# SCoulY/MuSCLe

Hardware: AMD Instinct MI355X
Metric: images/sec (whole node), MCL EfficientNet-B7 448x448 bs=32/GPU (higher is better)
Workload: dtype f32; 1 GPU; train_mcl.py loop body, step-A (epoch-4 gates: focal+softmargin+pairwise+ER+IMC, one backward, one Adam step), MuSCLe(efficientnet-b7, last_pooling=False, 21 classes), random-init weights; per_gpu_batch=32, global_batch=32, image=448x448, parallelism=single, optimizer=Adam(lr=1e-4, wd=5e-5) fused, launch=eager, weight-gradient GEMMs on a second stream

## Files before the change

### include/muscle_hip.h

```cpp
#ifndef MUSCLE_HIP_H
#define MUSCLE_HIP_H

#ifdef __cplusplus
extern "C" {
#endif

int mx_version(void);
int mx_abi_hash(void);
const char* mx_last_error(void);


int mx_pw_fwd_parts(int M, int N, int K);
int mx_pw_fwd(const float* A, int a_mode, const float* a_scale, const float* a_shift, const float* a_gate,
              int rows_per_sample, const float* W, float* C, int M, int K, int N, int lda, int ldc,
              const float* bias, const float* residual, int relu, float* stats, void* stream);

int mx_set_gemm_mode(int mode);
int mx_get_gemm_mode(void);
int mx_set_wgrad_kernel(int kernel, int groups);
int mx_get_wgrad_kernel(void);
int mx_gemm_uses_split(int kind, int M, int N, int K);

long mx_pw_planes_bytes(int N, int K);
int mx_pw_planes_tiles(int N, int K);
int mx_pw_planes_batch(const long* table, int n, int total_tiles, void* stream);
int mx_pw_fwd_uses_planes(int M, int K, int N);
int mx_pw_fwd_planes(const float* A, const void* Wplanes, float* C, int M, int K, int N, int lda, int ldc,
                     const float* bias, const float* residual, int relu, float* stats, void* stream);

int mx_transpose(const float* src, float* dst, int rows, int cols, void* stream);
int mx_transpose_batch(const long* table, int n, int total_tiles, void* stream);

int mx_pw_dgrad(const float* G, const float* W, float* dX, int M, int K, int N, int ldg, int ldx,
                const float* residual, void* stream);

int mx_pw_dgrad_bnbwd(const float* G, const float* X, const float* coef, const float* Wt, float* dX, float* dZ, int M, int K, int N,
                      int ldg, int ldx, const float* residual, void* stream);

int mx_pw_fwd_act_uses_planes(int M, int K, int N);
int mx_pw_fwd_planes_act(const float* A, const float* scale, const float* shift, const float* gate, int rows_per_sample,
                         const void* Wplanes, float* C, int M, int K, int N, int lda, int ldc, float* stats, void* stream);

int mx_pw_dgrad_bnbwd_planes(const float* G, const float* X, const float* coef, const void* WtPlanes, float* dX, int M, int K, int N,
                             int ldg, int ldx, const float* residual, void* stream);
int mx_pw_wgrad_tile_bnbwd_ok(int R, int Co, int Ci);
int mx_pw_wgrad_small_bnbwd_ok(int R, int Co, int Ci);
int mx_pw_wgrad_small_bnbwd(const float* G, const float* G2, const float* coef, const float* X, float* dW, int R, int Co, int Ci,
                            int ldg, int ldx, void* ws, long ws_bytes, void* stream);
int mx_pw_wgrad_tile_bnbwd(const float* G, const float* G2, const float* coef, const float* X, float* dW, int R, int Co, int Ci,
                           int ldg, int ldx, void* ws, long ws_bytes, void* stream);
int mx_pw_wgrad_tile_bnbwd_dz_ok(int R, int Co, int Ci, int ldg, int ldx);
int mx_pw_wgrad_tile_bnbwd_dz(const float* G, const float* G2, const float* coef, const float* X, float* dW, float* dz, int R, int Co,
                              int Ci, int ldg, int ldx, void* ws, long ws_bytes, void* stream);

long mx_pw_wgrad_ws(int R, int Co, int Ci);
int mx_pw_wgrad(const float* G, const float* X, int x_mode, const float* x_scale, const float* x_shift,
                const float* x_gate, int rows_per_sample, float* dW, int R, int Co, int Ci, int ldg, int ldx,
                void* ws, long ws_bytes, void* stream);

long mx_pw_wgrad_small_ws(int R, int Co, int Ci, int x_mode);
int mx_pw_wgrad_small(const float* G, const float* X, int x_mode, const float* x_scale, const float* x_shift,
                      const float* x_gate, int rows_per_sample, float* dW, int R, int Co, int Ci, int ldg, int ldx,
                      void* ws, long ws_bytes, void* stream);

long mx_pw_wgrad_tile_ws(int R, int Co, int Ci, int x_mode);
int mx_pw_wgrad_tile(const float* G, const float* X, int x_mode, const float* x_scale, const float* x_shift,
                     const float* x_gate, int rows_per_sample, float* dW, int R, int Co, int Ci, int ldg, int ldx,
                     void* ws, long ws_bytes, void* stream);

int mx_bgemm(int layout, const float* A, const float* B, float* C, int M, int N, int K, int lda, int ldb, int ldc,
             long sa, long sb, long sc, int batch, int relu, void* stream);


int mx_colreduce_parts(long rows, int C);
int mx_colstats(const float* X, long rows, int C, float* part, void* stream);

int mx_bn_finalize(const float* part, int P, int C, double count, const float* gamma, const float* beta, float* running_mean,
                   float* running_var, float momentum, float eps, int training, float* scale, float* shift,
                   float* mean, float* rstd, double* acc , void* stream);

int mx_fold_block(const float* We, const float* g0, const float* b0, const float* m0, const float* v0, float eps0,
                  const float* g1, const float* b1, const float* m1, const float* v1, float eps1,
                  const float* Wp, const float* g2, const float* b2, const float* m2, const float* v2, float eps2,
                  int Cin, int Cexp, int Cout, float* We_f, float* be, float* s1, float* t1, float* Wp_f, float* bp, void* stream);

int mx_bn_apply(const float* P, const float* scale, const float* shift, const float* row_scale, const float* residual,
                const float* gate, float* out, long rows, int C, int rows_per_sample, int act, void* stream);

int mx_bn_bwd_reduce(const float* G, const float* X, const float* row_scale, const float* gate, const float* gate_add,
                     const float* act_scale, const float* act_shift, long rows, int C, int rows_per_sample,
                     float* part, void* stream);

int mx_bn_bwd_finalize(const float* part, int P, int C, double count, const float* gamma, const float* mean, const float* rstd,
                       int training, float* dgamma, float* dbeta, float* c1, float* c2, float* c3, double* acc,
                       void* stream);

int mx_bn_bwd_apply(const float* G, const float* X, const float* row_scale, const float* gate, const float* gate_add,
                    const float* act_scale, const float* act_shift, const float* c1, const float* c2, const float* c3,
                    float* out, long rows, int C, int rows_per_sample, void* stream);

long mx_pool_ws(long rows, int C, int rows_per_sample, int planes);
int mx_pool_sum(const float* X, const float* G, const float* scale, const float* shift, int act, long rows, int C,
                int rows_per_sample, float* out, void* ws, long ws_bytes, void* stream);

int mx_se_bn1_pool(const float* dA, const float* X, const float* scale, const float* shift, long rows, int C, int rows_per_sample,
                   float* out5, void* ws, long ws_bytes, void* stream);
int mx_bn1_sums_finalize(const float* pooled5, const float* gate, const float* gh, const float* W1, float inv_hw, float* add,
                         int N, int C, int SQ, double count, const float* gamma, const float* mean, const float* rstd, int training,
                         float* dgamma, float* dbeta, float* c1, float* c2, float* c3, void* stream);


int mx_dwconv_fwd_parts(int N, int Ho, int Wo, int C, int S);
long mx_dwconv_fwd_ws(int N, int Ho, int Wo, int C, int S);
int mx_dwconv_fwd(const float* X, const float* scale, const float* shift, const float* W, float* Y, float* stats,
                  const float* pool_scale, const float* pool_shift, float* pooled, void* ws, long ws_bytes, int N,
                  int H, int Wd, int C, int K, int S, int pad_lo, int Ho, int Wo, void* stream);

int mx_dwconv_bwd_data(const float* dY, const float* W, const float* residual, float* dX, int N, int H, int Wd, int C,
                       int K, int S, int pad_lo, int Ho, int Wo, void* stream);

int mx_dwconv_bwd_weight_parts(int N, int Ho, int Wo, int C, int S);
int mx_dwconv_bwd_weight(const float* X, const float* scale, const float* shift, const float* dY, float* dW, float* dw_scratch,
                         int N, int H, int Wd, int C, int K, int S, int pad_lo, int Ho, int Wo, void* stream);

int mx_dwconv_bwd_fused_parts(int N, int H, int Wd, int C, int K);
int mx_dwconv_bwd_fused(const float* dA, const float* D, const float* gate, const float* add, const float* a1, const float* b1,
                        const float* c1, const float* c2, const float* c3, const float* X, const float* a0, const float* b0,
                        const float* W, const float* residual, float* gX, float* dW, float* dw_scratch, float* part, int N, int H,
                        int Wd, int C, int K, int pad_lo, void* stream);

int mx_dwconv_bwd_fused_bn0(const float* dA, const float* D, const float* gate, const float* add, const float* a1, const float* b1,
                            const float* c1, const float* c2, const float* c3, const float* X, const float* a0, const float* b0,
                            const float* W, float* gX, float* dW, float* dw_scratch, float* part, int N, int H, int Wd, int C, int K,
                            int pad_lo, void* ws, long ws_bytes, double count, const float* gamma, const float* mean, const float* rstd,
                            int training, float* dgamma, float* dbeta, float* o1, float* o2, float* o3, void* stream);

int mx_dwconv_bwd_fused_s2_parts(int N, int H, int Wd, int C, int K);
int mx_dwconv_bwd_fused_s2(const float* dA, const float* D, const float* gate, const float* add, const float* a1, const float* b1,
                           const float* c1, const float* c2, const float* c3, const float* X, const float* a0, const float* b0,
                           const float* W, float* gX, float* dW, float* dw_scratch, float* part, int N, int H, int Wd, int C, int K,
                           int pad_lo, int Ho, int Wo, void* stream);

int mx_dw_parts_reduce(const float* part, int P, int n, float* dW, void* stream);


int mx_se_fwd(const float* pooled_sum, float inv_hw, const float* W1, const float* b1, const float* W2, const float* b2,
              float* s, float* h, float* gate, int N, int C, int SQ, void* stream);

int mx_se_bwd(const float* ggate, const float* gate, const float* s, const float* h, const float* W2,
              float* dW1, float* db1, float* dW2, float* db2, float* gh, int N, int C,
              int SQ, void* stream);

int mx_se_bwd_gh(const float* ggate, const float* gate, const float* h, const float* W2, float* gh, int N, int C, int SQ,
                 void* stream);
int mx_se_bwd_params(const float* ggate, const float* gate, const float* s, const float* h, const float* gh, float* dW1, float* db1,
                     float* dW2, float* db2, int N, int C, int SQ, void* stream);

int mx_stem_im2col(const float* img, float* out, int N, int H, int W, int Ho, int Wo, int pad_lo, void* stream);


int mx_resize_nhwc(const float* src, float* dst, int N, int Hs, int Ws, int C, int Hd, int Wd, int ldd, int coff, int relu,
                   void* stream);

int mx_upsample_to_nchw(const float* src, float* dst, int N, int Hs, int Ws, int lds, int K, int Hd, int Wd, void* stream);

int mx_infer_accum(const float* src, float* acc, int h, int w, int lds, int K, int Hs, int Ws, int H, int W, int flip, void* stream);
int mx_infer_norm(float* acc, int channels, long HW, void* stream);

int mx_cam_infer(const long* passes, int npass, int lds, int K, int H, int W, const int* keep, int nkeep, float* out_cam,
                 float* out_sgc, void* stream);

int mx_seg_infer(const long* passes, int npass, int lds, int K, int H, int W, const float* cls_scale, unsigned char* pred,
                 float* prob, void* stream);
int mx_seg_confusion(const unsigned char* pred, const unsigned char* gt, int K, int H, int W, long long* counts, void* stream);

int mx_seg_infer_batch(const long* rows, int nrow, int B, int lds, int K, int H, int W, const float* cls_scale, unsigned char* pred,
                       float* prob, const unsigned char* gt, long long* counts, void* stream);

int mx_input_stage(const unsigned char* src, const int* jobs, float* dst, int n, int Hd, int Wd, void* stream);

int mx_color_jitter(unsigned char* src, const int* jobs, unsigned long long* sums, int n, int max_pixels, void* stream);
// ... 158 lines not shown
```

### muscle_amd/csrc/bn.hip

```cpp
#include "common.h"

struct ColGeom {
  int rows, C, c4;
  int tcols;
  int rpp;
  int rows_per_block;
  int rps;
};

static ColGeom col_geom(long rows, int C, int rps, long rows_limit ,
                        int groups = 1 , int planes = 1) {
  ColGeom g;
  g.rows = (int)rows; g.C = C; g.c4 = C / 4; g.rps = rps;
  {
    const int cand[] = {g.c4 <= 256 ? g.c4 : 256, 256, 192, 128, 96, 64, 48, 32};
    double best = -1.0;
    g.tcols = cand[0];
    for (int tc : cand) {
      if (tc > g.c4) continue;
      const double util = (double)g.c4 / (double)(cdiv(g.c4, tc) * tc) * (double)(256 / tc * tc) / 256.0;
      if (groups > 1 ? util > best - 1e-9 : util > best + 1e-9) { best = util; g.tcols = tc; }
    }
  }
  g.rpp = 256 / g.tcols;
// ... 145 lines not shown
}

template <class F, int NOUT, bool PER_SAMPLE, typename OutT>
static void launch_colreduce(const F& f, long rows, int C, int rps, OutT* o0, OutT* o1, hipStream_t st, void* ws = nullptr) {
  if (PER_SAMPLE) {
    dim3 grid;
    ColGeom g = pool_geom(rows, C, rps, &grid);
    hipLaunchKernelGGL((colreduce_kernel<F, NOUT, PER_SAMPLE, OutT>), grid, dim3(256), 0, st, f, g, o0, o1,
                       ws ? reinterpret_cast<float*>((char*)ws + MX_WS_COUNTER_BYTES) : nullptr, reinterpret_cast<unsigned*>(ws));
    return;
  }
  ColGeom g = col_geom(rows, C, rps, rows, 1);
  dim3 grid(cdiv(rows, g.rows_per_block), cdiv(g.c4, g.tcols), 1);
  hipLaunchKernelGGL((colreduce_kernel<F, NOUT, PER_SAMPLE, OutT>), grid, dim3(256), 0, st, f, g, o0, o1, (float*)nullptr, (unsigned*)nullptr);
}

struct GEff {
  const float* G; const float* X;
  const float* rs; const float* gate; const float* add;
  const float* a; const float* b;
  int C, rps;
  __device__ __forceinline__ void get(long r, int c, float4& g, float4& x) const {
    get_n(r, (int)((unsigned)r / (unsigned)rps), c, g, x);
  }
  __device__ __forceinline__ void get_n(long r, int n, int c, float4& g, float4& x) const {
    g = ld4(G + r * C + c);
    x = ld4(X + r * C + c);
    if (rs) { float s = rs[n]; g.x *= s; g.y *= s; g.z *= s; g.w *= s; }
    if (gate) {
      float4 gt = ld4(gate + (long)n * C + c), ad = ld4(add + (long)n * C + c);
      g.x = g.x * gt.x + ad.x; g.y = g.y * gt.y + ad.y; g.z = g.z * gt.z + ad.z; g.w = g.w * gt.w + ad.w;
    }
    if (a) {
      float4 aa = ld4(a + c), bb = ld4(b + c);
      g.x *= swish_gradf_(aa.x * x.x + bb.x); g.y *= swish_gradf_(aa.y * x.y + bb.y);
      g.z *= swish_gradf_(aa.z * x.z + bb.z); g.w *= swish_gradf_(aa.w * x.w + bb.w);
    }
  }
};

struct FBwdReduce {
  static constexpr bool kPipelined = false;
  GEff e;
  __device__ __forceinline__ void eval(long r, int c, float4& s0, float4& s1) const {
    float4 g, x;
    e.get(r, c, g, x);
    s0.x += g.x; s0.y += g.y; s0.z += g.z; s0.w += g.w;
    s1.x += g.x * x.x; s1.y += g.y * x.y; s1.z += g.z * x.z; s1.w += g.w * x.w;
  }
};

struct FStats {
  static constexpr bool kPipelined = false;
  const float* X; int C;
  __device__ __forceinline__ void eval(long r, int c, float4& s0, float4& s1) const {
    float4 x = ld4(X + r * C + c);
    s0.x += x.x; s0.y += x.y; s0.z += x.z; s0.w += x.w;
    s1.x += x.x * x.x; s1.y += x.y * x.y; s1.z += x.z * x.z; s1.w += x.w * x.w;
  }
};

struct FPool {
  static constexpr bool kPipelined = true;
  const float* X; const float* G; const float* a; const float* b; int C; int act;
  __device__ __forceinline__ float4 value(float4 x, int c) const {
    if (a) {
      float4 aa = ld4(a + c), bb = ld4(b + c);
      x.x = aa.x * x.x + bb.x; x.y = aa.y * x.y + bb.y; x.z = aa.z * x.z + bb.z; x.w = aa.w * x.w + bb.w;
    }
    if (act) { x.x = swishf_(x.x); x.y = swishf_(x.y); x.z = swishf_(x.z); x.w = swishf_(x.w); }
    return x;
  }
  __device__ __forceinline__ void eval(long r, int c, float4& s0, float4& s1) const {
    float4 x = value(ld4(X + r * C + c), c);
    if (G) {
      float4 g = ld4(G + r * C + c);
      x.x *= g.x; x.y *= g.y; x.z *= g.z; x.w *= g.w;
    }
    s0.x += x.x; s0.y += x.y; s0.z += x.z; s0.w += x.w;
  }
};

__global__ __launch_bounds__(256) void se_bn1_pool_kernel(const float* G, const float* X, const float* a, const float* b, ColGeom g,
                                                          float* out , long plane, float* scratch ,
                                                          unsigned* counters) {
  __shared__ float4 sm[5][256];
  __shared__ unsigned last_flag;
  const int tid = threadIdx.x;
  const int used = g.tcols * g.rpp;
  const int tc = tid % g.tcols, tr = tid / g.tcols;
  const int c4 = blockIdx.y * g.tcols + tc;
  const int sample = blockIdx.z;
  const long r0 = (long)sample * g.rps + (long)blockIdx.x * g.rows_per_block;
  const long r1 = min((long)(sample + 1) * g.rps, r0 + g.rows_per_block);
  float4 acc[5];
#pragma unroll
  for (int i = 0; i < 5; ++i) acc[i] = make_float4(0, 0, 0, 0);
  if (tid < used && c4 < g.c4) {
    const int c = 4 * c4;
    const float4 aa = ld4(a + c), bb = ld4(b + c);
#define SE1(f, x, ga)                                          \
      {                                                           \
        float z = aa.f * x.f + bb.f, sg = sigmoidf_(z);           \
        float act = z * sg, sp = sg * (1.f + z * (1.f - sg));     \
        acc[0].f += ga.f * act; acc[1].f += ga.f * sp; acc[2].f += sp; \
        acc[3].f += ga.f * sp * x.f; acc[4].f += sp * x.f;        \
      }
    long r = r0 + tr;
    for (; r + 3 * g.rpp < r1; r += 4 * g.rpp) {
      const float4 x0 = ld4(X + r * g.C + c), g0 = ld4(G + r * g.C + c);
      const float4 x1 = ld4(X + (r + g.rpp) * g.C + c), g1 = ld4(G + (r + g.rpp) * g.C + c);
      const float4 x2 = ld4(X + (r + 2 * g.rpp) * g.C + c), g2 = ld4(G + (r + 2 * g.rpp) * g.C + c);
      const float4 x3 = ld4(X + (r + 3 * g.rpp) * g.C + c), g3 = ld4(G + (r + 3 * g.rpp) * g.C + c);
      SE1(x, x0, g0) SE1(y, x0, g0) SE1(z, x0, g0) SE1(w, x0, g0)
      SE1(x, x1, g1) SE1(y, x1, g1) SE1(z, x1, g1) SE1(w, x1, g1)
      SE1(x, x2, g2) SE1(y, x2, g2) SE1(z, x2, g2) SE1(w, x2, g2)
      SE1(x, x3, g3) SE1(y, x3, g3) SE1(z, x3, g3) SE1(w, x3, g3)
    }
    for (; r + g.rpp < r1; r += 2 * g.rpp) {
      const float4 x0 = ld4(X + r * g.C + c), g0 = ld4(G + r * g.C + c);
      const float4 x1 = ld4(X + (r + g.rpp) * g.C + c), g1 = ld4(G + (r + g.rpp) * g.C + c);
      SE1(x, x0, g0) SE1(y, x0, g0) SE1(z, x0, g0) SE1(w, x0, g0)
      SE1(x, x1, g1) SE1(y, x1, g1) SE1(z, x1, g1) SE1(w, x1, g1)
    }
    for (; r < r1; r += g.rpp) {
      const float4 x0 = ld4(X + r * g.C + c), g0 = ld4(G + r * g.C + c);
      SE1(x, x0, g0) SE1(y, x0, g0) SE1(z, x0, g0) SE1(w, x0, g0)
    }
#undef SE1
  }
#pragma unroll
  for (int i = 0; i < 5; ++i) sm[i][tid] = acc[i];
  __syncthreads();
  const bool owner = tid < g.tcols && c4 < g.c4;
  const long off = (long)sample * g.C + 4 * c4;
  float* dst = gridDim.x == 1 ? out : scratch + (long)blockIdx.x * 5 * plane;
  if (owner) {
#pragma unroll
    for (int i = 0; i < 5; ++i) {
      float4 s0 = sm[i][tid];
      for (int k = 1; k < g.rpp; ++k) { float4 t0 = sm[i][tid + k * g.tcols]; s0.x += t0.x; s0.y += t0.y; s0.z += t0.z; s0.w += t0.w; }
      if (gridDim.x == 1) st4(dst + i * plane + off, s0);
      else mx_st4_wt(dst + i * plane + off, s0);
    }
  }
  if (gridDim.x == 1) return;
  if (!mx_last_arriver(counters + sample * gridDim.y + blockIdx.y, gridDim.x, &last_flag)) return;
  if (owner) {
#pragma unroll
    for (int i = 0; i < 5; ++i) st4(out + i * plane + off, ordered_sum4(scratch + i * plane + off, gridDim.x, 5 * plane));
  }
}

constexpr int BN_MAX_SLICES = 64;
__global__ __launch_bounds__(256) void bn_parts_reduce_kernel(const float* part, int P, int C, int rows_per_slice, double* acc) {
  __shared__ double sh[2][8][32];
  const int cl = threadIdx.x & 31, rl = threadIdx.x >> 5;
  const int c = blockIdx.x * 32 + cl;
  const int p0 = blockIdx.y * rows_per_slice, p1 = min(P, p0 + rows_per_slice);
  double a = 0.0, b = 0.0;
  if (c < C) {
    int p = p0 + rl;
    for (; p + 24 < p1; p += 32) {
      float a0 = part[(long)p * 2 * C + c], b0 = part[(long)p * 2 * C + C + c];
      float a1 = part[(long)(p + 8) * 2 * C + c], b1 = part[(long)(p + 8) * 2 * C + C + c];
      float a2 = part[(long)(p + 16) * 2 * C + c], b2 = part[(long)(p + 16) * 2 * C + C + c];
      float a3 = part[(long)(p + 24) * 2 * C + c], b3 = part[(long)(p + 24) * 2 * C + C + c];
      a += ((double)a0 + (double)a1) + ((double)a2 + (double)a3);
      b += ((double)b0 + (double)b1) + ((double)b2 + (double)b3);
    }
    for (; p < p1; p += 8) { a += (double)part[(long)p * 2 * C + c]; b += (double)part[(long)p * 2 * C + C + c]; }
  }
  sh[0][rl][cl] = a; sh[1][rl][cl] = b;
  __syncthreads();
  if (rl != 0 || c >= C) return;
  for (int i = 1; i < 8; ++i) { a += sh[0][i][cl]; b += sh[1][i][cl]; }
  acc[(long)blockIdx.y * 2 * C + c] = a;
  acc[(long)blockIdx.y * 2 * C + C + c] = b;
}

static int launch_parts_reduce(const float* part, int P, int C, double* acc, hipStream_t st) {
  int slices = P / 32;
  if (slices < 1) slices = 1;
  if (slices > BN_MAX_SLICES) slices = BN_MAX_SLICES;
  int rps = (P + slices - 1) / slices;
  slices = (P + rps - 1) / rps;
  hipLaunchKernelGGL(bn_parts_reduce_kernel, dim3(cdiv(C, 32), slices), dim3(256), 0, st, part, P, C, rps, acc);
  return slices;
}

struct BnFwdFin {
  double count; const float* gamma; const float* beta; float* rmean; float* rvar; float momentum, eps; int training;
  float* scale; float* shift; float* mean_out; float* rstd_out;
};

__device__ __forceinline__ void bn_fwd_finalize_one(int c, double st0, double st1, double count, const float* gamma,
                                                    const float* beta, float* rmean, float* rvar, float momentum, float eps,
                                                    int training, float* scale, float* shift, float* mean_out, float* rstd_out) {
  float mean, rstd;
  if (training) {
    double m = st0 / count;
    double var = st1 / count - m * m;
    if (var < 0) var = 0;
    mean = (float)m;
    rstd = (float)(1.0 / sqrt(var + (double)eps));
    double unb = count > 1 ? var * count / (count - 1) : var;
    rmean[c] = (1.f - momentum) * rmean[c] + momentum * mean;
    rvar[c] = (1.f - momentum) * rvar[c] + momentum * (float)unb;
  } else {
    mean = rmean[c];
    rstd = 1.0f / sqrtf(rvar[c] + eps);
  }
  float sc = gamma[c] * rstd;
  scale[c] = sc;
  shift[c] = beta[c] - mean * sc;
  mean_out[c] = mean;
  rstd_out[c] = rstd;
}

__device__ __forceinline__ bool slices_sum(const double* acc, int slices, int C, double& s0, double& s1) {
  __shared__ double sh[2][8][32];
  const int cl = threadIdx.x & 31, sl = threadIdx.x >> 5;
  const int c = blockIdx.x * 32 + cl;
  s0 = s1 = 0.0;
  if (c < C)
    for (int i = sl; i < slices; i += 8) { s0 += acc[(long)i * 2 * C + c]; s1 += acc[(long)i * 2 * C + C + c]; }
  sh[0][sl][cl] = s0; sh[1][sl][cl] = s1;
  __syncthreads();
  if (sl != 0 || c >= C) return false;
  for (int i = 1; i < 8; ++i) { s0 += sh[0][i][cl]; s1 += sh[1][i][cl]; }
  return true;
}

__global__ __launch_bounds__(256) void bn_finalize_kernel(const double* acc, int slices, int C, double count, const float* gamma,
                                   const float* beta, float* rmean, float* rvar, float momentum, float eps, int training,
                                   float* scale, float* shift, float* mean_out, float* rstd_out) {
  double st0, st1;
  if (!slices_sum(acc, training ? slices : 0, C, st0, st1)) return;
  const int c = blockIdx.x * 32 + (threadIdx.x & 31);
  bn_fwd_finalize_one(c, st0, st1, count, gamma, beta, rmean, rvar, momentum, eps, training, scale, shift, mean_out, rstd_out);
}


__global__ __launch_bounds__(256) void bn_bwd_finalize_kernel(const double* acc, int slices, int C, double count, const float* gamma,
                                       const float* mean, const float* rstd, int training, float* dgamma, float* dbeta,
                                       float* c1, float* c2, float* c3) {
  double s0, s1;
  if (!slices_sum(acc, slices, C, s0, s1)) return;
  const int c = blockIdx.x * 32 + (threadIdx.x & 31);
  bn_bwd_finalize_one(c, s0, s1, count, gamma, mean, rstd, training, dgamma, dbeta, c1, c2, c3);
}

constexpr int FUSED_FINALIZE_MAX_ROWS = 1024;
template <bool BWD>
__global__ __launch_bounds__(256) void bn_reduce_finalize_kernel(const float* part, int P, int C, BnFwdFin f, BnBwdFin b) {
  __shared__ double sh[2][8][32];
  const int cl = threadIdx.x & 31, rl = threadIdx.x >> 5;
  const int c = blockIdx.x * 32 + cl;
  double s0 = 0.0, s1 = 0.0;
  if (c < C) bn_parts_lane_sum(part, P, C, c, rl, s0, s1);
  sh[0][rl][cl] = s0; sh[1][rl][cl] = s1;
  __syncthreads();
  if (rl != 0 || c >= C) return;
  for (int i = 1; i < 8; ++i) { s0 += sh[0][i][cl]; s1 += sh[1][i][cl]; }
  if (BWD) bn_bwd_finalize_one(c, s0, s1, b.count, b.gamma, b.mean, b.rstd, b.training, b.dgamma, b.dbeta, b.c1, b.c2, b.c3);
  else bn_fwd_finalize_one(c, s0, s1, f.count, f.gamma, f.beta, f.rmean, f.rvar, f.momentum, f.eps, 1, f.scale, f.shift, f.mean_out, f.rstd_out);
}

constexpr int B1_NL = 16;
template <bool STAGED>
__global__ __launch_bounds__(64 * B1_NL) void bn1_sums_finalize_kernel(const float* pooled , const float* gate, const float* gh,
                                                                      const float* W1, float inv_hw, float* add, int N, int C, int SQ,
                                                                      BnBwdFin b) {
  extern __shared__ float smem_b1[];
  const int cl = threadIdx.x & 63, nl = threadIdx.x >> 6;
  const int c = blockIdx.x * 64 + cl;
  const float* ghs = STAGED ? smem_b1 : gh;
  if (STAGED) {
    for (int i = threadIdx.x; i < N * SQ; i += 64 * B1_NL) smem_b1[i] = gh[i];
    __syncthreads();
  }
  const long plane = (long)N * C;
  double s0 = 0.0, s1 = 0.0;
  if (c < C) {
    for (int n0 = nl; n0 < N; n0 += 2 * B1_NL) {
      const int n1 = n0 + B1_NL;
      float a0 = 0.f, a1 = 0.f;
      const float* g0 = ghs + n0 * SQ;
      const float* g1 = ghs + (n1 < N ? n1 : n0) * SQ;
      int j = 0;
      for (; j + 32 <= SQ; j += 32) {
        float w[32];
#pragma unroll
        for (int u = 0; u < 32; ++u) w[u] = W1[(long)(j + u) * C + c];
        __builtin_amdgcn_sched_barrier(0);
#pragma unroll
        for (int u = 0; u < 32; ++u) { a0 += g0[j + u] * w[u]; a1 += g1[j + u] * w[u]; }
      }
      for (; j + 8 <= SQ; j += 8) {
        float w[8];
#pragma unroll
        for (int u = 0; u < 8; ++u) w[u] = W1[(long)(j + u) * C + c];
        __builtin_amdgcn_sched_barrier(0);
#pragma unroll
        for (int u = 0; u < 8; ++u) { a0 += g0[j + u] * w[u]; a1 += g1[j + u] * w[u]; }
      }
// ... 86 lines not shown
  float eps0, eps1, eps2;
  int Cin, Cexp, Cout;
  float *We_f, *be, *s1, *t1, *Wp_f, *bp;
};
__global__ __launch_bounds__(256) void fold_block_kernel(FoldArgs a) {
  const long tid = (long)blockIdx.x * 256 + threadIdx.x, nth = (long)gridDim.x * 256;
  if (a.We) {
    for (long i = tid; i < (long)a.Cexp * a.Cin; i += nth) {
      const int c = (int)(i / a.Cin);
      a.We_f[i] = a.We[i] * (a.g0[c] * rsqrtf(a.v0[c] + a.eps0));
    }
    for (long c = tid; c < a.Cexp; c += nth) {
      const float s = a.g0[c] * rsqrtf(a.v0[c] + a.eps0);
      a.be[c] = a.b0[c] - s * a.m0[c];
    }
  }
  for (long c = tid; c < a.Cexp; c += nth) {
    const float s = a.g1[c] * rsqrtf(a.v1[c] + a.eps1);
    a.s1[c] = s; a.t1[c] = a.b1[c] - s * a.m1[c];
  }
  for (long i = tid; i < (long)a.Cout * a.Cexp; i += nth) {
    const int c = (int)(i / a.Cexp);
    a.Wp_f[i] = a.Wp[i] * (a.g2[c] * rsqrtf(a.v2[c] + a.eps2));
  }
  for (long c = tid; c < a.Cout; c += nth) {
    const float s = a.g2[c] * rsqrtf(a.v2[c] + a.eps2);
    a.bp[c] = a.b2[c] - s * a.m2[c];
  }
}

extern "C" {

int mx_fold_block(const float* We, const float* g0, const float* b0, const float* m0, const float* v0, float eps0,
                  const float* g1, const float* b1, const float* m1, const float* v1, float eps1,
                  const float* Wp, const float* g2, const float* b2, const float* m2, const float* v2, float eps2,
                  int Cin, int Cexp, int Cout, float* We_f, float* be, float* s1, float* t1, float* Wp_f, float* bp, void* stream) {
  MX_CHECK_ARG(Cin > 0 && Cexp > 0 && Cout > 0, "fold_block: bad extents");
  MX_CHECK_ARG(!We || (g0 && b0 && m0 && v0 && We_f && be), "fold_block: expand weight without its BatchNorm / outputs");
  MX_CHECK_ARG(g1 && b1 && m1 && v1 && s1 && t1 && Wp && g2 && b2 && m2 && v2 && Wp_f && bp, "fold_block: null pointer");
  FoldArgs a{We, g0, b0, m0, v0, g1, b1, m1, v1, Wp, g2, b2, m2, v2, eps0, eps1, eps2, Cin, Cexp, Cout, We_f, be, s1, t1, Wp_f, bp};
  long work = (long)Cexp * (Cin > Cout ? Cin : Cout);
  int grid = (int)((work + 1023) / 1024);
  if (grid > 1024) grid = 1024;
  if (grid < 1) grid = 1;
  hipLaunchKernelGGL(fold_block_kernel, dim3(grid), dim3(256), 0, (hipStream_t)stream, a);
  MX_LAUNCH_CHECK();
  return MX_OK;
}

int mx_colreduce_parts(long rows, int C) {
  if (rows <= 0 || C <= 0 || C % 4) return MX_EARG;
  return colreduce_parts(rows, C);
}

int mx_colstats(const float* X, long rows, int C, float* part, void* stream) {
  MX_CHECK_ARG(X && part && rows > 0 && C > 0 && C % 4 == 0, "colstats: bad args rows=%ld C=%d", rows, C);
  FStats f{X, C};
  launch_colreduce<FStats, 2, false, float>(f, rows, C, 1, part, part, (hipStream_t)stream);
  MX_LAUNCH_CHECK();
  return MX_OK;
}

int mx_bn_finalize(const float* part, int P, int C, double count, const float* gamma, const float* beta, float* running_mean,
                   float* running_var, float momentum, float eps, int training, float* scale, float* shift,
                   float* mean, float* rstd, double* acc, void* stream) {
  MX_CHECK_ARG(C > 0 && gamma && beta && running_mean && running_var && scale && shift && mean && rstd,
               "bn_finalize: null argument");
  MX_CHECK_ARG(!training || (part && P > 0 && count > 0 && acc), "bn_finalize: training needs partial statistics, count and acc[64][2C]");
  if (training && P <= FUSED_FINALIZE_MAX_ROWS) {
    BnFwdFin f{count, gamma, beta, running_mean, running_var, momentum, eps, 1, scale, shift, mean, rstd};
    hipLaunchKernelGGL(bn_reduce_finalize_kernel<false>, dim3(cdiv(C, 32)), dim3(256), 0, (hipStream_t)stream, part, P, C, f, BnBwdFin{});
    MX_LAUNCH_CHECK();
    return MX_OK;
  }
  int slices = 0;
  if (training) slices = launch_parts_reduce(part, P, C, acc, (hipStream_t)stream);
  hipLaunchKernelGGL(bn_finalize_kernel, dim3(cdiv(C, 32)), dim3(256), 0, (hipStream_t)stream, acc, slices, C, count, gamma,
                     beta, running_mean, running_var, momentum, eps, training, scale, shift, mean, rstd);
  MX_LAUNCH_CHECK();
  return MX_OK;
}

int mx_bn_apply(const float* P, const float* scale, const float* shift, const float* row_scale, const float* residual,
                const float* gate, float* out, long rows, int C, int rows_per_sample, int act, void* stream) {
  MX_CHECK_ARG(P && scale && shift && out && rows > 0 && C % 4 == 0 && rows_per_sample > 0, "bn_apply: bad args");
  long total4 = rows * (C / 4);
  hipLaunchKernelGGL(bn_apply_kernel, dim3(grid_for(total4)), dim3(256), 0, (hipStream_t)stream, P, scale, shift,
                     row_scale, residual, gate, out, total4, C, rows_per_sample, act);
  MX_LAUNCH_CHECK();
  return MX_OK;
}

int mx_bn_bwd_reduce(const float* G, const float* X, const float* row_scale, const float* gate, const float* gate_add,
                     const float* act_scale, const float* act_shift, long rows, int C, int rows_per_sample,
                     float* part, void* stream) {
  MX_CHECK_ARG(G && X && part && rows > 0 && C % 4 == 0 && rows_per_sample > 0, "bn_bwd_reduce: bad args");
  MX_CHECK_ARG((gate == nullptr) == (gate_add == nullptr), "bn_bwd_reduce: gate and gate_add come together");
  MX_CHECK_ARG((act_scale == nullptr) == (act_shift == nullptr), "bn_bwd_reduce: act scale/shift come together");
  FBwdReduce f{GEff{G, X, row_scale, gate, gate_add, act_scale, act_shift, C, rows_per_sample}};
  launch_colreduce<FBwdReduce, 2, false, float>(f, rows, C, rows_per_sample, part, part, (hipStream_t)stream);
  MX_LAUNCH_CHECK();
  return MX_OK;
}

int mx_bn_bwd_finalize(const float* part, int P, int C, double count, const float* gamma, const float* mean, const float* rstd,
                       int training, float* dgamma, float* dbeta, float* c1, float* c2, float* c3, double* acc, void* stream) {
  MX_CHECK_ARG(part && P > 0 && gamma && mean && rstd && dgamma && dbeta && c1 && c2 && c3 && acc && C > 0 && count > 0,
               "bn_bwd_finalize: bad args");
  if (P <= FUSED_FINALIZE_MAX_ROWS) {
    BnBwdFin b{count, gamma, mean, rstd, training, dgamma, dbeta, c1, c2, c3};
    hipLaunchKernelGGL(bn_reduce_finalize_kernel<true>, dim3(cdiv(C, 32)), dim3(256), 0, (hipStream_t)stream, part, P, C, BnFwdFin{}, b);
    MX_LAUNCH_CHECK();
    return MX_OK;
  }
  const int slices = launch_parts_reduce(part, P, C, acc, (hipStream_t)stream);
  hipLaunchKernelGGL(bn_bwd_finalize_kernel, dim3(cdiv(C, 32)), dim3(256), 0, (hipStream_t)stream, acc, slices, C, count, gamma,
                     mean, rstd, training, dgamma, dbeta, c1, c2, c3);
  MX_LAUNCH_CHECK();
  return MX_OK;
}

int mx_bn_bwd_apply(const float* G, const float* X, const float* row_scale, const float* gate, const float* gate_add,
                    const float* act_scale, const float* act_shift, const float* c1, const float* c2, const float* c3,
                    float* out, long rows, int C, int rows_per_sample, void* stream) {
  MX_CHECK_ARG(G && X && out && c1 && c2 && c3 && rows > 0 && C % 4 == 0 && rows_per_sample > 0, "bn_bwd_apply: bad args");
  GEff e{G, X, row_scale, gate, gate_add, act_scale, act_shift, C, rows_per_sample};
  long total4 = rows * (C / 4);
  hipLaunchKernelGGL(bn_bwd_apply_kernel, dim3(grid_for(total4)), dim3(256), 0, (hipStream_t)stream, e, c1, c2, c3, out,
                     total4);
  MX_LAUNCH_CHECK();
  return MX_OK;
}

long mx_pool_ws(long rows, int C, int rows_per_sample, int planes) {
  if (rows <= 0 || C <= 0 || C % 4 || rows_per_sample <= 0 || rows % rows_per_sample || (planes != 1 && planes != 5)) return MX_EARG;
  return pool_ws_bytes(rows, C, rows_per_sample, planes);
}

int mx_se_bn1_pool(const float* dA, const float* X, const float* scale, const float* shift, long rows, int C, int rows_per_sample,
                   float* out5, void* ws, long ws_bytes, void* stream) {
  MX_CHECK_ARG(dA && X && scale && shift && out5 && rows > 0 && C % 4 == 0 && rows_per_sample > 0 && rows % rows_per_sample == 0,
               "se_bn1_pool: bad args");
  const int N = (int)(rows / rows_per_sample);
  dim3 grid;
  ColGeom g = pool_geom(rows, C, rows_per_sample, &grid, 5);
  const long need = pool_ws_bytes(rows, C, rows_per_sample, 5);
  MX_CHECK_ARG(need == 0 || (ws && ws_bytes >= need && ((uintptr_t)ws & 15) == 0), "se_bn1_pool: workspace of %ld bytes required (mx_pool_ws)", need);
  hipLaunchKernelGGL(se_bn1_pool_kernel, grid, dim3(256), 0, (hipStream_t)stream, dA, X, scale, shift, g, out5, (long)N * C,
                     need ? reinterpret_cast<float*>((char*)ws + MX_WS_COUNTER_BYTES) : nullptr, reinterpret_cast<unsigned*>(ws));
  MX_LAUNCH_CHECK();
  return MX_OK;
}

int mx_bn1_sums_finalize(const float* pooled5, const float* gate, const float* gh, const float* W1, float inv_hw, float* add,
                         int N, int C, int SQ, double count, const float* gamma, const float* mean, const float* rstd, int training,
                         float* dgamma, float* dbeta, float* c1, float* c2, float* c3, void* stream) {
  MX_CHECK_ARG(pooled5 && gate && gh && W1 && add && N > 0 && C > 0 && SQ > 0 && count > 0, "bn1_sums_finalize: bad args");
  MX_CHECK_ARG(gamma && mean && rstd && dgamma && dbeta && c1 && c2 && c3, "bn1_sums_finalize: null pointer");
  const size_t redb = 2 * B1_NL * 64 * sizeof(double);
  const size_t shb = (size_t)((N * SQ + 1) & ~1) * sizeof(float) + redb;
  BnBwdFin b{count, gamma, mean, rstd, training, dgamma, dbeta, c1, c2, c3};
  if (shb <= 64 * 1024)
    hipLaunchKernelGGL(bn1_sums_finalize_kernel<true>, dim3(cdiv(C, 64)), dim3(64 * B1_NL), shb, (hipStream_t)stream, pooled5, gate, gh, W1,
                       inv_hw, add, N, C, SQ, b);
  else
    hipLaunchKernelGGL(bn1_sums_finalize_kernel<false>, dim3(cdiv(C, 64)), dim3(64 * B1_NL), redb, (hipStream_t)stream, pooled5, gate, gh, W1,
                       inv_hw, add, N, C, SQ, b);
  MX_LAUNCH_CHECK();
  return MX_OK;
}

int mx_pool_sum(const float* X, const float* G, const float* scale, const float* shift, int act, long rows, int C,
                int rows_per_sample, float* out, void* ws, long ws_bytes, void* stream) {
  MX_CHECK_ARG(X && out && rows > 0 && C % 4 == 0 && rows_per_sample > 0 && rows % rows_per_sample == 0,
               "pool_sum: bad args rows=%ld C=%d rps=%d", rows, C, rows_per_sample);
  const long need = pool_ws_bytes(rows, C, rows_per_sample, 1);
  MX_CHECK_ARG(need == 0 || (ws && ws_bytes >= need && ((uintptr_t)ws & 15) == 0), "pool_sum: workspace of %ld bytes required (mx_pool_ws)", need);
  FPool f{X, G, scale, shift, C, act};
  launch_colreduce<FPool, 1, true, float>(f, rows, C, rows_per_sample, out, out, (hipStream_t)stream, need ? ws : nullptr);
  MX_LAUNCH_CHECK();
  return MX_OK;
}

}
```

### muscle_amd/csrc/gemm.hip

```cpp
#include "common.h"
#include <type_traits>
#include <stdlib.h>

typedef float f32x16 __attribute__((ext_vector_type(16)));
typedef float f32x4 __attribute__((ext_vector_type(4)));

struct GemmArgs {
  MxOperand a, b;
  float* c;
  int M, N, K;
  int lda, ldb, ldc;
  long sa, sb, sc;
  const float* bias;
  const float* residual;
  int relu;
  float* stats;
  int ksplit;
  int xcd_nt;
  int mt, zt;
  unsigned long long* stamps;
  float* a_out;
  float* ws;
};

#ifndef MX_GEMM_STAMP
#define MX_GEMM_STAMP(g, slot)
#endif
static unsigned long long* mx_gemm_stamps = nullptr;

enum { L_NT = 0, L_NN = 1, L_TN = 2 };

template <int ROWS, int PAD, int BK>
struct SlabK {
  static constexpr int TOTAL = ROWS * (BK / 4);
  static constexpr int PER = (TOTAL + 255) / 256;
  float4 v[PER];
  __device__ __forceinline__ void load(const MxOperand& o, const float* base, int ld, int r0, int rows_total,
                                       int k0, int K, int tid) {
#pragma unroll
    for (int i = 0; i < PER; ++i) {
      int idx = tid + 256 * i;
      int k4 = idx % (BK / 4), row = idx / (BK / 4);
      int r = r0 + row, k = k0 + 4 * k4;
      float4 x = make_float4(0.f, 0.f, 0.f, 0.f);
      if (idx < TOTAL && r < rows_total && k < K) {
        x = ld4(base + (long)r * ld + k);
        x = mx_apply(o, x, r, k, K);
      }
      v[i] = x;
    }
  }
  __device__ __forceinline__ void store(float* lds, int tid) const {
#pragma unroll
    for (int i = 0; i < PER; ++i) {
      int idx = tid + 256 * i;
      int k4 = idx % (BK / 4), row = idx / (BK / 4);
      if (idx < TOTAL) {
        float* p = lds + (4 * k4) * (ROWS + PAD) + row;
        p[0] = v[i].x; p[ROWS + PAD] = v[i].y; p[2 * (ROWS + PAD)] = v[i].z; p[3 * (ROWS + PAD)] = v[i].w;
      }
    }
  }
};

template <int COLS, int PAD, int BK>
struct SlabN {
  static constexpr int C4 = COLS / 4;
  static constexpr int TOTAL = BK * C4;
  static constexpr int PER = (TOTAL + 255) / 256;
  float4 v[PER];
  __device__ __forceinline__ void load(const MxOperand& o, const float* base, int ld, int c0, int cols_total,
                                       int k0, int Kdim, int tid) {
#pragma unroll
    for (int i = 0; i < PER; ++i) {
      int idx = tid + 256 * i;
      int c4 = idx % C4, kk = idx / C4;
      int k = k0 + kk, c = c0 + 4 * c4;
      float4 x = make_float4(0.f, 0.f, 0.f, 0.f);
      if (idx < TOTAL && k < Kdim && c < cols_total) {
        x = ld4(base + (long)k * ld + c);
        x = mx_apply(o, x, k, c, cols_total);
      }
      v[i] = x;
    }
  }
  __device__ __forceinline__ void store(float* lds, int tid) const {
#pragma unroll
    for (int i = 0; i < PER; ++i) {
      int idx = tid + 256 * i;
      int c4 = idx % C4, kk = idx / C4;
      if (idx < TOTAL) st4(lds + kk * (COLS + PAD) + 4 * c4, v[i]);
    }
  }
};

constexpr int gemm_min_waves(int acc_regs, int bk) { return (acc_regs == 64 && bk == 16) ? 4 : 1; }

template <int LAYOUT, int WM, int WN, int TM, int TN, int BK>
__global__ __launch_bounds__(256, gemm_min_waves(TM * TN * 16, BK)) void gemm_kernel(GemmArgs g) {
  constexpr int BM = WM * TM * 32, BN = WN * TN * 32;
  constexpr int PADA = (LAYOUT == L_TN) ? 4 : 1;
  constexpr int PADB = (LAYOUT == L_NT) ? 1 : 4;
  constexpr int SA = BM + PADA, SB = BN + PADB;
  __shared__ __attribute__((aligned(16))) float smem[2 * BK * SA + 2 * BK * SB];
  float* As = smem;
  float* Bs = smem + 2 * BK * SA;

  const int tid = threadIdx.x, lane = tid & 63, wave = tid >> 6;
  const int l31 = lane & 31, h = lane >> 5;
  const int wm = wave / WN, wn = wave % WN;
  int tile_m = blockIdx.x, tile_n = blockIdx.y;
  int zz = blockIdx.z;
  if (LAYOUT == L_TN && g.xcd_nt > 0) {
    const int L = blockIdx.x, xcd = L & 7, j = L >> 3;
    const int tiles = g.mt * g.xcd_nt;
    const int t = j % tiles;
    zz = (j / tiles) * 8 + xcd;
    if (zz >= g.zt) return;
    tile_m = t % g.mt; tile_n = t / g.mt;
  } else if (g.xcd_nt > 0) {
    const int L = blockIdx.x, xcd = L & 7, j = L >> 3;
    tile_n = j % g.xcd_nt;
    tile_m = (j / g.xcd_nt) * 8 + xcd;
    if (tile_m >= g.mt) return;
  }
  const int m0 = tile_m * BM, n0 = tile_n * BN;
  const int z = zz;

  const float* A = g.a.p;
  const float* B = g.b.p;
  float* C = g.c;
  int kbeg = 0, kend = g.K;
  if (LAYOUT == L_TN) {
    kbeg = z * g.ksplit;
    kend = min(g.K, kbeg + g.ksplit);
    C += z * g.sc;
  } else {
    A += z * g.sa; B += z * g.sb; C += z * g.sc;
  }

  f32x16 acc[TM][TN];
#pragma unroll
  for (int i = 0; i < TM; ++i)
#pragma unroll
    for (int j = 0; j < TN; ++j)
#pragma unroll
      for (int r = 0; r < 16; ++r) acc[i][j][r] = 0.f;

  typename std::conditional<LAYOUT == L_TN, SlabN<BM, PADA, BK>, SlabK<BM, PADA, BK>>::type sa;
  typename std::conditional<LAYOUT == L_NT, SlabK<BN, PADB, BK>, SlabN<BN, PADB, BK>>::type sb;

  auto load = [&](int k0) {
    if constexpr (LAYOUT == L_TN) sa.load(g.a, A, g.lda, m0, g.M, k0, kend, tid);
    else sa.load(g.a, A, g.lda, m0, g.M, k0, kend, tid);
    if constexpr (LAYOUT == L_NT) sb.load(g.b, B, g.ldb, n0, g.N, k0, kend, tid);
    else sb.load(g.b, B, g.ldb, n0, g.N, k0, kend, tid);
  };

  MX_GEMM_STAMP(g, 0);
  const int nk = (kend - kbeg + BK - 1) / BK;
  if (nk > 0) {
    load(kbeg);
    sa.store(As, tid);
    sb.store(Bs, tid);
    if (nk > 1) load(kbeg + BK);
  }
  __syncthreads();
  MX_GEMM_STAMP(g, 1);
  for (int kt = 0; kt < nk; ++kt) {
    const int cur = kt & 1;
    if (kt + 1 < nk) {
      sa.store(As + (cur ^ 1) * BK * SA, tid);
      sb.store(Bs + (cur ^ 1) * BK * SB, tid);
      if (kt + 2 < nk) load(kbeg + (kt + 2) * BK);
    }
// ... 26 lines not shown

  MX_GEMM_STAMP(g, 2);
  float csum[TN], csq[TN];
#pragma unroll
  for (int j = 0; j < TN; ++j) csum[j] = csq[j] = 0.f;
#pragma unroll
  for (int j = 0; j < TN; ++j) {
    const int col = n0 + wn * TN * 32 + j * 32 + l31;
    const bool cok = col < g.N;
    const float bias = (g.bias && cok) ? g.bias[col] : 0.f;
#pragma unroll
    for (int i = 0; i < TM; ++i) {
#pragma unroll
      for (int r = 0; r < 16; ++r) {
        const int row = m0 + wm * TM * 32 + i * 32 + (r & 3) + 8 * (r >> 2) + 4 * h;
        if (cok && row < g.M) {
          float v = acc[i][j][r];
          const long idx = (long)row * g.ldc + col;
          if (LAYOUT == L_TN) {
            unsafeAtomicAdd(C + idx, v);
          } else {
            v += bias;
            if (g.residual) v += g.residual[idx];
            if (g.relu) v = fmaxf(v, 0.f);
            __builtin_nontemporal_store(v, C + idx);
            csum[j] += v;
            csq[j] += v * v;
          }
        }
      }
    }
  }
  if (LAYOUT != L_TN && g.stats) {
    float* red = smem;
#pragma unroll
    for (int j = 0; j < TN; ++j) {
      float s = csum[j] + __shfl_xor(csum[j], 32, 64);
      float q = csq[j] + __shfl_xor(csq[j], 32, 64);
      if (h == 0) {
        red[(wm * 2 + 0) * BN + wn * TN * 32 + j * 32 + l31] = s;
        red[(wm * 2 + 1) * BN + wn * TN * 32 + j * 32 + l31] = q;
      }
    }
    __syncthreads();
    float* prow = g.stats + (long)tile_m * 2 * g.N;
    for (int i = tid; i < 2 * BN; i += 256) {
      const int which = i / BN, col = i - which * BN;
      float v = 0.f;
#pragma unroll
      for (int w = 0; w < WM; ++w) v += red[(w * 2 + which) * BN + col];
      if (n0 + col < g.N) prow[which * g.N + n0 + col] = v;
    }
  }
  MX_GEMM_STAMP(g, 3);
}

template <int LAYOUT, int WM, int WN, int TM, int TN, int BK = 16>
static void launch(const GemmArgs& g, int batch_or_splits, hipStream_t st) {
  constexpr int BM = WM * TM * 32, BN = WN * TN * 32;
  const int mt = cdiv(g.M, BM), nt = cdiv(g.N, BN);
  if (LAYOUT != L_TN && nt >= 2 && nt <= 16 && mt >= 64) {
    GemmArgs a = g;
    a.xcd_nt = nt; a.mt = mt;
    dim3 grid(8 * cdiv(mt, 8) * nt, 1, batch_or_splits);
    hipLaunchKernelGGL((gemm_kernel<LAYOUT, WM, WN, TM, TN, BK>), grid, dim3(256), 0, st, a);
    return;
  }
  if (LAYOUT == L_TN && batch_or_splits >= 8 && mt * nt >= 2 && mt * nt <= 8 && g.K >= 200000 && g.K < 1000000) {
    GemmArgs a = g;
    a.xcd_nt = nt; a.mt = mt; a.zt = batch_or_splits;
    dim3 grid(8 * cdiv(batch_or_splits, 8) * mt * nt, 1, 1);
    hipLaunchKernelGGL((gemm_kernel<LAYOUT, WM, WN, TM, TN, BK>), grid, dim3(256), 0, st, a);
    return;
  }
  GemmArgs a = g;
  a.xcd_nt = 0; a.mt = mt; a.zt = batch_or_splits;
  dim3 grid(mt, nt, batch_or_splits);
  hipLaunchKernelGGL((gemm_kernel<LAYOUT, WM, WN, TM, TN, BK>), grid, dim3(256), 0, st, a);
}

struct TileCfg { int bm, bn; };
static const TileCfg kCfgs[] = {
    {128, 128},
    {128, 96},
    {128, 32},
    {256, 64},
    {128, 64},
    {128, 128},
    {128, 64},
    {128, 64},
    {128, 32},
    {128, 96},
    {256, 128},
    {128, 256},
};
constexpr int kNumCfgs = sizeof(kCfgs) / sizeof(kCfgs[0]);

static int pick_cfg(int layout, int M, int N, int K) {
  (void)K;
  if (const char* e = getenv("MX_GEMM_CFG")) {
    int forced = atoi(e);
    if (forced >= 0 && forced < kNumCfgs) return forced;
  }
  if (layout == L_TN) {
    if (N >= 384 && N % 128 == 0) return 0;
    if (N % 96 == 0) return 1;
    return 2;
  }
  static const struct { int cfg; double eff; } cand[] = {{0, 1.00}, {1, 0.97}, {4, 0.95}, {2, 0.85}};
  int best = 2;
  double best_score = -1.0;
  for (const auto& c : cand) {
    const TileCfg t = kCfgs[c.cfg];
    const long nt = cdiv(N, t.bn), tiles = (long)cdiv(M, t.bm) * nt;
    const double pad = (double)N / (double)(nt * t.bn);
    const double per_cu = (double)tiles / 256.0;
    const double balance = per_cu / (double)(long)(per_cu + 0.999999);
    if (c.cfg == 4 && N % 64 != 0) continue;
    double score = c.eff * pad * balance;
    if (per_cu < 2.0) score *= 0.85;
    if (score > best_score + 1e-9) { best_score = score; best = c.cfg; }
  }
  return best;
}

template <int LAYOUT>
static void dispatch(const GemmArgs& g, int zdim, hipStream_t st) {
  switch (pick_cfg(LAYOUT, g.M, g.N, g.K)) {
    case 0: launch<LAYOUT, 2, 2, 2, 2>(g, zdim, st); break;
    case 1: launch<LAYOUT, 4, 1, 1, 3>(g, zdim, st); break;
    case 2: launch<LAYOUT, 4, 1, 1, 1>(g, zdim, st); break;
    case 3: launch<LAYOUT, 4, 1, 2, 2>(g, zdim, st); break;
    case 4: launch<LAYOUT, 4, 1, 1, 2>(g, zdim, st); break;
    case 5: launch<LAYOUT, 2, 2, 2, 2, 32>(g, zdim, st); break;
    case 6: launch<LAYOUT, 2, 2, 2, 1>(g, zdim, st); break;
    case 7: launch<LAYOUT, 2, 2, 2, 1, 32>(g, zdim, st); break;
    case 8: launch<LAYOUT, 4, 1, 1, 1, 32>(g, zdim, st); break;
    case 9: launch<LAYOUT, 4, 1, 1, 3, 32>(g, zdim, st); break;
    case 10: launch<LAYOUT, 2, 2, 4, 2>(g, zdim, st); break;
    default: launch<LAYOUT, 2, 2, 2, 4>(g, zdim, st); break;
  }
}


static __device__ __forceinline__ float row16_sum(float v) {
  v += __int_as_float(__builtin_amdgcn_update_dpp(0, __float_as_int(v), 0x128, 0xf, 0xf, false));
  v += __int_as_float(__builtin_amdgcn_update_dpp(0, __float_as_int(v), 0x124, 0xf, 0xf, false));
  v += __int_as_float(__builtin_amdgcn_update_dpp(0, __float_as_int(v), 0x122, 0xf, 0xf, false));
  v += __int_as_float(__builtin_amdgcn_update_dpp(0, __float_as_int(v), 0x121, 0xf, 0xf, false));
  return v;
}

template <int WM, int WN, int TM, int TN>
static __device__ __forceinline__ void nt_epilogue(const GemmArgs& g, float* C, int tile_m, int m0, int n0, f32x4 (&acc)[TM][TN],
                                                   float* smem, int tid) {
  constexpr int BN = WN * TN * 16;
  const int lane = tid & 63, wave = tid >> 6;
  const int l15 = lane & 15, q = lane >> 4;
  const int wm = wave / WN, wn = wave % WN;
  float* red = smem;
  const bool vec = ((g.ldc | g.N) & 3) == 0;
  f32x4 cs[TN], cq[TN];
#pragma unroll
  for (int j = 0; j < TN; ++j) cs[j] = cq[j] = f32x4{0.f, 0.f, 0.f, 0.f};
  const bool lean = vec && !g.bias && !g.relu && m0 + WM * TM * 16 <= g.M && n0 + BN <= g.N;
  if (lean) {
    const long idx0 = (long)(m0 + wm * TM * 16 + l15) * g.ldc + n0 + wn * TN * 16 + 4 * q;
    float* cp = C + idx0;
    const long istep = 16L * g.ldc;
    if (g.residual) {
      const float* rp = g.residual + idx0;
#pragma unroll
      for (int j = 0; j < TN; ++j)
#pragma unroll
        for (int i = 0; i < TM; ++i) {
          const f32x4 v = acc[i][j] + *reinterpret_cast<const f32x4*>(rp + i * istep + 16 * j);
          cs[j] += v; cq[j] += v * v;
          __builtin_nontemporal_store(v, reinterpret_cast<f32x4*>(cp + i * istep + 16 * j));
        }
    } else if (g.stats) {
#pragma unroll
      for (int j = 0; j < TN; ++j)
#pragma unroll
        for (int i = 0; i < TM; ++i) {
          const f32x4 v = acc[i][j];
          cs[j] += v; cq[j] += v * v;
          __builtin_nontemporal_store(v, reinterpret_cast<f32x4*>(cp + i * istep + 16 * j));
        }
    } else {
#pragma unroll
      for (int j = 0; j < TN; ++j)
#pragma unroll
        for (int i = 0; i < TM; ++i)
          __builtin_nontemporal_store(acc[i][j], reinterpret_cast<f32x4*>(cp + i * istep + 16 * j));
    }
  } else
#pragma unroll
  for (int j = 0; j < TN; ++j) {
    const int col = n0 + wn * TN * 16 + 16 * j + 4 * q;
    const bool full = vec && col + 3 < g.N;
    float b[4] = {0.f, 0.f, 0.f, 0.f};
    if (g.bias) {
#pragma unroll
      for (int e = 0; e < 4; ++e) if (col + e < g.N) b[e] = g.bias[col + e];
    }
#pragma unroll
    for (int i = 0; i < TM; ++i) {
      const int row = m0 + wm * TM * 16 + 16 * i + l15;
      if (row >= g.M || col >= g.N) continue;
      const long idx = (long)row * g.ldc + col;
      float v[4] = {acc[i][j][0] + b[0], acc[i][j][1] + b[1], acc[i][j][2] + b[2], acc[i][j][3] + b[3]};
      if (g.residual) {
        if (full) {
          const float4 r4 = ld4(g.residual + idx);
          v[0] += r4.x; v[1] += r4.y; v[2] += r4.z; v[3] += r4.w;
        } else {
#pragma unroll
          for (int e = 0; e < 4; ++e) if (col + e < g.N) v[e] += g.residual[idx + e];
        }
      }
      if (g.relu) {
#pragma unroll
        for (int e = 0; e < 4; ++e) v[e] = fmaxf(v[e], 0.f);
      }
#pragma unroll
      for (int e = 0; e < 4; ++e) {
        const float u = (col + e < g.N) ? v[e] : 0.f;
        cs[j][e] += u; cq[j][e] += u * u;
      }
      if (full) {
        f32x4 o = {v[0], v[1], v[2], v[3]};
        __builtin_nontemporal_store(o, reinterpret_cast<f32x4*>(C + idx));
      } else {
#pragma unroll
        for (int e = 0; e < 4; ++e) if (col + e < g.N) C[idx + e] = v[e];
      }
    }
  }
  MX_GEMM_STAMP(g, 7);
  if (g.stats) {
#pragma unroll
    for (int j = 0; j < TN; ++j) {
      f32x4 s, sq;
#pragma unroll
      for (int e = 0; e < 4; ++e) { s[e] = row16_sum(cs[j][e]); sq[e] = row16_sum(cq[j][e]); }
      if (l15 == 0) {
        *reinterpret_cast<f32x4*>(red + (wm * 2 + 0) * BN + wn * TN * 16 + 16 * j + 4 * q) = s;
        *reinterpret_cast<f32x4*>(red + (wm * 2 + 1) * BN + wn * TN * 16 + 16 * j + 4 * q) = sq;
      }
    }
    __syncthreads();
    float* prow = g.stats + (long)tile_m * 2 * g.N;
    for (int i = tid; i < 2 * BN; i += 256) {
      const int which = i / BN, col = i - which * BN;
      float v = 0.f;
#pragma unroll
      for (int w = 0; w < WM; ++w) v += red[(w * 2 + which) * BN + col];
      if (n0 + col < g.N) prow[which * g.N + n0 + col] = v;
    }
  }
}

template <int AMODE>
static __device__ __forceinline__ float4 nt_prologue(float4 v, float4 sc, float4 sh, float4 gt) {
  if (AMODE == MX_PLAIN) return v;
  v.x = sc.x * v.x + sh.x; v.y = sc.y * v.y + sh.y; v.z = sc.z * v.z + sh.z; v.w = sc.w * v.w + sh.w;
  if (AMODE == MX_BNACT) {
    v.x = swishf_(v.x) * gt.x; v.y = swishf_(v.y) * gt.y; v.z = swishf_(v.z) * gt.z; v.w = swishf_(v.w) * gt.w;
  }
  return v;
}

constexpr int gemm_nt_waves(int acc) { return acc <= 48 ? 4 : acc <= 64 ? 3 : 2; }

template <int WM, int WN, int TM, int TN, int AMODE>
__global__ __launch_bounds__(256, gemm_nt_waves(TM * TN * 4 + (AMODE == MX_BNBWD ? 16 : 0))) void gemm_nt_kernel(GemmArgs g) {
  constexpr int BM = WM * TM * 16, BN = WN * TN * 16, LS = 20;
  constexpr int PA = (BM * 4 + 255) / 256, PB = (BN * 4 + 255) / 256;
  constexpr int SMEM = 2 * (BM + BN) * LS;
  static_assert(WM * WN == 4, "four waves");
  static_assert(WM * 2 * BN <= SMEM, "statistics staging does not fit the operand buffers");
  __shared__ __attribute__((aligned(16))) float smem[SMEM];
  const int tid = threadIdx.x, lane = tid & 63, wave = tid >> 6;
  const int l15 = lane & 15, q = lane >> 4;
  const int wm = wave / WN, wn = wave % WN;
  int tile_m = blockIdx.x, tile_n = blockIdx.y;
  if (g.xcd_nt > 0) {
    const int L = blockIdx.x, xcd = L & 7, j = L >> 3;
    tile_n = j % g.xcd_nt;
    tile_m = (j / g.xcd_nt) * 8 + xcd;
    if (tile_m >= g.mt) return;
  }
  const int m0 = tile_m * BM, n0 = tile_n * BN;
  const long zb = blockIdx.z;
  const float* A = g.a.p + zb * g.sa;
  const float* B = g.b.p + zb * g.sb;
  float* C = g.c + zb * g.sc;
  const int K = g.K;

  const int ck = (tid & 3) * 4;
  float4 ra[PA], rb[PB];
  float4 gt[(AMODE == MX_BNACT || AMODE == MX_BNBWD) ? PA : 1];
  float4 sc4 = make_float4(0.f, 0.f, 0.f, 0.f), sh4 = sc4;
  float4 c34 = sc4;
  long ga_off[AMODE == MX_BNACT ? PA : 1];
  const float* pa[PA];
  const float* pb[PB];
  bool oka[PA], okb[PB];
#pragma unroll
  for (int i = 0; i < PA; ++i) {
    const int row = (tid + 256 * i) >> 2;
    oka[i] = (tid + 256 * i) < BM * 4 && m0 + row < g.M;
    pa[i] = A + (long)(m0 + row) * g.lda + ck;
    if (AMODE == MX_BNACT) ga_off[i] = g.a.rowp ? (long)((m0 + row) / g.a.rps) * K + ck : -1;
  }
#pragma unroll
  for (int i = 0; i < PB; ++i) {
    const int row = (tid + 256 * i) >> 2;
    okb[i] = (tid + 256 * i) < BN * 4 && n0 + row < g.N;
    pb[i] = B + (long)(n0 + row) * g.ldb + ck;
  }
  auto load = [&](int k0) {
    const bool kin = k0 + ck < K;
#pragma unroll
    for (int i = 0; i < PA; ++i) {
      ra[i] = (oka[i] && kin) ? ld4(pa[i] + k0) : make_float4(0.f, 0.f, 0.f, 0.f);
      if (AMODE == MX_BNACT) gt[i] = (oka[i] && kin && ga_off[i] >= 0) ? ld4(g.a.rowp + ga_off[i] + k0) : make_float4(1.f, 1.f, 1.f, 1.f);
      if (AMODE == MX_BNBWD) gt[i] = (oka[i] && kin) ? ld4(g.a.rowp + (pa[i] - g.a.p) + k0) : make_float4(0.f, 0.f, 0.f, 0.f);
    }
    if (AMODE != MX_PLAIN) {
      sc4 = kin ? ld4(g.a.c1 + k0 + ck) : make_float4(0.f, 0.f, 0.f, 0.f);
      sh4 = kin ? ld4(g.a.c2 + k0 + ck) : make_float4(0.f, 0.f, 0.f, 0.f);
      if (AMODE == MX_BNBWD) c34 = kin ? ld4(g.a.c1 + 2 * K + k0 + ck) : make_float4(0.f, 0.f, 0.f, 0.f);
    }
#pragma unroll
    for (int i = 0; i < PB; ++i) rb[i] = (okb[i] && kin) ? ld4(pb[i] + k0) : make_float4(0.f, 0.f, 0.f, 0.f);
  };
  auto store = [&](float* As, float* Bs, int k0) {
    const bool kin = k0 + ck < K;
#pragma unroll
    for (int i = 0; i < PA; ++i) {
      if ((tid + 256 * i) < BM * 4) {
        float4 v = ra[i];
        if (AMODE == MX_BNBWD) {
          if (oka[i] && kin) {
            const float4 x = gt[AMODE == MX_BNBWD ? i : 0];
            v.x = sc4.x * v.x + sh4.x * x.x + c34.x; v.y = sc4.y * v.y + sh4.y * x.y + c34.y;
            v.z = sc4.z * v.z + sh4.z * x.z + c34.z; v.w = sc4.w * v.w + sh4.w * x.w + c34.w;
            if (tile_n == 0) st4(g.a_out + (pa[i] - g.a.p) + k0, v);
          }
        } else if (AMODE != MX_PLAIN && oka[i] && kin) v = nt_prologue<AMODE>(v, sc4, sh4, gt[AMODE == MX_BNACT ? i : 0]);
        st4(As + ((tid + 256 * i) >> 2) * LS + ck, v);
      }
    }
#pragma unroll
    for (int i = 0; i < PB; ++i)
      if ((tid + 256 * i) < BN * 4) st4(Bs + ((tid + 256 * i) >> 2) * LS + ck, rb[i]);
  };

  f32x4 acc[TM][TN];
#pragma unroll
  for (int i = 0; i < TM; ++i)
#pragma unroll
    for (int j = 0; j < TN; ++j) acc[i][j] = f32x4{0.f, 0.f, 0.f, 0.f};

  float* As0 = smem;
  float* Bs0 = smem + 2 * BM * LS;
  MX_GEMM_STAMP(g, 0);
  const int nk = (K + 15) / 16;
  load(0);
  store(As0, Bs0, 0);
  if (nk > 1) load(16);
  __syncthreads();
  MX_GEMM_STAMP(g, 1);
  for (int kt = 0; kt < nk; ++kt) {
    const int cur = kt & 1;
    if (kt + 1 < nk) {
      store(As0 + (cur ^ 1) * BM * LS, Bs0 + (cur ^ 1) * BN * LS, (kt + 1) * 16);
      if (kt + 2 < nk) load((kt + 2) * 16);
    }
    const float* as = As0 + cur * BM * LS + (wm * TM * 16 + l15) * LS + 4 * q;
    const float* bs = Bs0 + cur * BN * LS + (wn * TN * 16 + l15) * LS + 4 * q;
    f32x4 av[TM], bv[TN];
#pragma unroll
    for (int i = 0; i < TM; ++i) av[i] = *reinterpret_cast<const f32x4*>(as + 16 * LS * i);
#pragma unroll
    for (int j = 0; j < TN; ++j) bv[j] = *reinterpret_cast<const f32x4*>(bs + 16 * LS * j);
#pragma unroll
    for (int st = 0; st < 4; ++st)
#pragma unroll
      for (int i = 0; i < TM; ++i)
#pragma unroll
        for (int j = 0; j < TN; ++j)
          acc[i][j] = __builtin_amdgcn_mfma_f32_16x16x4f32(bv[j][st], av[i][st], acc[i][j], 0, 0, 0);
    __syncthreads();
  }
  MX_GEMM_STAMP(g, 2);
  nt_epilogue<WM, WN, TM, TN>(g, C, tile_m, m0, n0, acc, smem, tid);
  MX_GEMM_STAMP(g, 3);
}

typedef __bf16 bf16x8 __attribute__((ext_vector_type(8)));

static __device__ __forceinline__ void split3_pair(float x0, float x1, unsigned& h, unsigned& m, unsigned& l) {
  const unsigned u0 = __float_as_uint(x0) & 0xffff0000u, u1 = __float_as_uint(x1) & 0xffff0000u;
  const float r0 = x0 - __uint_as_float(u0), r1 = x1 - __uint_as_float(u1);
  const unsigned v0 = __float_as_uint(r0) & 0xffff0000u, v1 = __float_as_uint(r1) & 0xffff0000u;
  const float s0 = r0 - __uint_as_float(v0), s1 = r1 - __uint_as_float(v1);
  h = __builtin_amdgcn_perm(u1, u0, 0x07060302u);
  m = __builtin_amdgcn_perm(v1, v0, 0x07060302u);
  l = __builtin_amdgcn_perm(__float_as_uint(s1), __float_as_uint(s0), 0x07060302u);
}

template <int AMODE, int NJ>
__global__ __launch_bounds__(256, NJ == 4 ? 2 : 3) void gemm_nt_split_kernel(GemmArgs g) {
  constexpr int BM = 128, BN = 64 * NJ, WN = 2, WNC = 32 * NJ;
  constexpr int PA_ = 128 * 32, PB_ = BN * 32;
  constexpr int STAGE = 3 * PA_ + 3 * PB_;
  constexpr int PS = WNC + 4;
  constexpr int SMEM = (2 * STAGE > 4 * 32 * PS * 4 + 2 * 2 * BN * 4) ? 2 * STAGE : 4 * 32 * PS * 4 + 2 * 2 * BN * 4;
  __shared__ __attribute__((aligned(16))) unsigned char smem[SMEM];
  const int tid = threadIdx.x, lane = tid & 63, wave = tid >> 6;
  const int l31 = lane & 31, hf = lane >> 5;
  const int wm = wave / WN, wn = wave % WN;
  int tile_m = blockIdx.x, tile_n = blockIdx.y;
  if (g.xcd_nt > 0) {
    const int L = blockIdx.x, xcd = L & 7, j = L >> 3;
    tile_n = j % g.xcd_nt;
    tile_m = (j / g.xcd_nt) * 8 + xcd;
    if (tile_m >= g.mt) return;
  }
  const int m0 = tile_m * BM, n0 = tile_n * BN;
  const long zb = blockIdx.z;
  const float* A = g.a.p + zb * g.sa;
  const float* B = g.b.p + zb * g.sb;
  float* C = g.c + zb * g.sc;
  const int K = g.K;

  constexpr int NB = BN / 64;
  const int ck = (tid & 3) * 4;
  float4 ra[2], rb[NB];
  float4 gt[AMODE == MX_BNACT ? 2 : 1];
  float4 sc4 = make_float4(0.f, 0.f, 0.f, 0.f), sh4 = sc4;
  long ga_off[AMODE == MX_BNACT ? 2 : 1];
  const float* pa[2];
  const float* pb[NB];
  bool oka[2], okb[NB];
  int woff[2];
#pragma unroll
  for (int i = 0; i < 2; ++i) {
    const int row = (tid >> 2) + 64 * i;
    oka[i] = m0 + row < g.M;
    pa[i] = A + (long)(m0 + row) * g.lda + ck;
    if (AMODE == MX_BNACT) ga_off[i] = g.a.rowp ? (long)((m0 + row) / g.a.rps) * K + ck : -1;
    if (i < NB) {
      okb[i] = n0 + row < g.N;
      pb[i] = B + (long)(n0 + row) * g.ldb + ck;
    }
    const int kq = tid & 3;
    woff[i] = row * 32 + (((kq >> 1) ^ ((row >> 3) & 1)) << 4) + ((kq & 1) << 3);
  }
  auto load = [&](int k0) {
    const bool kin = k0 + ck < K;
#pragma unroll
    for (int i = 0; i < 2; ++i) {
      ra[i] = (oka[i] && kin) ? ld4(pa[i] + k0) : make_float4(0.f, 0.f, 0.f, 0.f);
      if (AMODE == MX_BNACT) gt[i] = (oka[i] && kin && ga_off[i] >= 0) ? ld4(g.a.rowp + ga_off[i] + k0) : make_float4(1.f, 1.f, 1.f, 1.f);
      if (i < NB) rb[i] = (okb[i] && kin) ? ld4(pb[i] + k0) : make_float4(0.f, 0.f, 0.f, 0.f);
    }
    if (AMODE != MX_PLAIN) {
      sc4 = kin ? ld4(g.a.c1 + k0 + ck) : make_float4(0.f, 0.f, 0.f, 0.f);
      sh4 = kin ? ld4(g.a.c2 + k0 + ck) : make_float4(0.f, 0.f, 0.f, 0.f);
    }
  };
  auto put = [&](unsigned char* base, int plane, int off, float4 v) {
    unsigned h0, m0_, l0, h1, m1, l1;
    split3_pair(v.x, v.y, h0, m0_, l0);
    split3_pair(v.z, v.w, h1, m1, l1);
    *reinterpret_cast<uint2*>(base + off) = make_uint2(h0, h1);
    *reinterpret_cast<uint2*>(base + plane + off) = make_uint2(m0_, m1);
    *reinterpret_cast<uint2*>(base + 2 * plane + off) = make_uint2(l0, l1);
  };
  auto store = [&](unsigned char* st, int k0) {
    const bool kin = k0 + ck < K;
#pragma unroll
    for (int i = 0; i < 2; ++i) {
      float4 v = ra[i];
      if (AMODE != MX_PLAIN && oka[i] && kin) v = nt_prologue<AMODE>(v, sc4, sh4, gt[AMODE == MX_BNACT ? i : 0]);
      put(st, PA_, woff[i], v);
      if (i < NB) put(st + 3 * PA_, PB_, woff[i], rb[i]);
    }
  };

  f32x16 acc[2][NJ];
#pragma unroll
  for (int i = 0; i < 2; ++i)
#pragma unroll
    for (int j = 0; j < NJ; ++j)
#pragma unroll
      for (int r = 0; r < 16; ++r) acc[i][j][r] = 0.f;

  int fa[2], fb[NJ];
#pragma unroll
  for (int i = 0; i < 2; ++i) {
    const int ra_ = wm * 64 + 32 * i + l31;
    fa[i] = ra_ * 32 + ((hf ^ ((ra_ >> 3) & 1)) << 4);
  }
#pragma unroll
  for (int j = 0; j < NJ; ++j) {
    const int rb_ = wn * WNC + 32 * j + l31;
    fb[j] = rb_ * 32 + ((hf ^ ((rb_ >> 3) & 1)) << 4);
  }
  const int nk = (K + 15) / 16;
  load(0);
  store(smem, 0);
  if (nk > 1) load(16);
  __syncthreads();
  for (int kt = 0; kt < nk; ++kt) {
    const int cur = kt & 1;
    if (kt + 1 < nk) {
      store(smem + (cur ^ 1) * STAGE, (kt + 1) * 16);
      if (kt + 2 < nk) load((kt + 2) * 16);
    }
    const unsigned char* sa = smem + cur * STAGE;
    const unsigned char* sb = sa + 3 * PA_;
    bf16x8 av[2][3], bv[NJ][3];
#pragma unroll
    for (int p = 0; p < 3; ++p) {
#pragma unroll
      for (int i = 0; i < 2; ++i) av[i][p] = *reinterpret_cast<const bf16x8*>(sa + p * PA_ + fa[i]);
#pragma unroll
      for (int j = 0; j < NJ; ++j) bv[j][p] = *reinterpret_cast<const bf16x8*>(sb + p * PB_ + fb[j]);
    }
    constexpr int PW[6] = {0, 2, 1, 0, 1, 0}, PX[6] = {2, 0, 1, 1, 0, 0};
#pragma unroll
    for (int t = 0; t < 6; ++t)
#pragma unroll
      for (int i = 0; i < 2; ++i)
#pragma unroll
        for (int j = 0; j < NJ; ++j)
          acc[i][j] = __builtin_amdgcn_mfma_f32_32x32x16_bf16(bv[j][PW[t]], av[i][PX[t]], acc[i][j], 0, 0, 0);
    __syncthreads();
  }
  float* patch = reinterpret_cast<float*>(smem) + wave * (32 * PS);
  float* red = reinterpret_cast<float*>(smem) + 4 * 32 * PS;
  const bool vec = ((g.ldc | g.N) & 3) == 0;
  f32x4 cs[NJ][4], cq[NJ][4];
#pragma unroll
  for (int j = 0; j < NJ; ++j)
#pragma unroll
    for (int gq = 0; gq < 4; ++gq) cs[j][gq] = cq[j][gq] = f32x4{0.f, 0.f, 0.f, 0.f};
#pragma unroll
  for (int i = 0; i < 2; ++i) {
    const int rbase = m0 + wm * 64 + 32 * i;
    const int row = rbase + l31;
#pragma unroll
    for (int j = 0; j < NJ; ++j)
#pragma unroll
      for (int gq = 0; gq < 4; ++gq) {
        const int cl = 32 * j + 8 * gq + 4 * hf;
        const int col = n0 + wn * WNC + cl;
        float v[4];
#pragma unroll
        for (int e = 0; e < 4; ++e) v[e] = acc[i][j][4 * gq + e] + ((g.bias && col + e < g.N) ? g.bias[col + e] : 0.f);
        if (g.residual && row < g.M) {
          const long idx = (long)row * g.ldc + col;
          if (vec && col + 3 < g.N) {
            const float4 r4 = ld4(g.residual + idx);
            v[0] += r4.x; v[1] += r4.y; v[2] += r4.z; v[3] += r4.w;
          } else {
#pragma unroll
            for (int e = 0; e < 4; ++e) if (col + e < g.N) v[e] += g.residual[idx + e];
          }
        }
        if (g.relu) {
#pragma unroll
          for (int e = 0; e < 4; ++e) v[e] = fmaxf(v[e], 0.f);
        }
        if (row < g.M) {
#pragma unroll
          for (int e = 0; e < 4; ++e) {
            const float u = (col + e < g.N) ? v[e] : 0.f;
            cs[j][gq][e] += u; cq[j][gq][e] += u * u;
          }
        }
        *reinterpret_cast<f32x4*>(patch + l31 * PS + cl) = f32x4{v[0], v[1], v[2], v[3]};
      }
    constexpr int C4 = WNC / 4, RPP = 64 / C4;
#pragma unroll
    for (int t = 0; t < 32 / RPP; ++t) {
      const int rl = t * RPP + lane / C4, c4 = (lane % C4) * 4;
      const int orow = rbase + rl, ocol = n0 + wn * WNC + c4;
      const float4 v4 = ld4(patch + rl * PS + c4);
      if (orow < g.M && ocol < g.N) {
        const long idx = (long)orow * g.ldc + ocol;
        if (vec && ocol + 3 < g.N) {
          __builtin_nontemporal_store(f32x4{v4.x, v4.y, v4.z, v4.w}, reinterpret_cast<f32x4*>(C + idx));
        } else {
          const float v[4] = {v4.x, v4.y, v4.z, v4.w};
#pragma unroll
          for (int e = 0; e < 4; ++e) if (ocol + e < g.N) C[idx + e] = v[e];
        }
      }
    }
  }
  if (g.stats) {
#pragma unroll
    for (int j = 0; j < NJ; ++j)
#pragma unroll
      for (int gq = 0; gq < 4; ++gq) {
        f32x4 s, sq;
#pragma unroll
        for (int e = 0; e < 4; ++e) {
          float a = row16_sum(cs[j][gq][e]), q = row16_sum(cq[j][gq][e]);
          a += __shfl_xor(a, 16, 64); q += __shfl_xor(q, 16, 64);
          s[e] = a; sq[e] = q;
        }
        if (l31 == 0) {
          const int coll = wn * WNC + 32 * j + 8 * gq + 4 * hf;
          *reinterpret_cast<f32x4*>(red + (wm * 2 + 0) * BN + coll) = s;
          *reinterpret_cast<f32x4*>(red + (wm * 2 + 1) * BN + coll) = sq;
        }
      }
    __syncthreads();
    float* prow = g.stats + (long)tile_m * 2 * g.N;
    for (int i = tid; i < 2 * BN; i += 256) {
      const int which = i / BN, col = i - which * BN;
      const float v = red[(0 * 2 + which) * BN + col] + red[(1 * 2 + which) * BN + col];
      if (n0 + col < g.N) prow[which * g.N + n0 + col] = v;
    }
  }
}

static __device__ __forceinline__ int swz_w(int row) { return ((row >> 3) & 1) * 3; }

static __device__ __forceinline__ void glds16(const void* src, void* lds_wave_base) {
  __builtin_amdgcn_global_load_lds((const __attribute__((address_space(1))) void*)src,
                                   (__attribute__((address_space(3))) void*)lds_wave_base, 16, 0, 0);
}

__global__ __launch_bounds__(256) void split_planes_kernel(const long* __restrict__ table, int njobs) {
  __shared__ int job_s;
  if (threadIdx.x == 0) {
    int j = 0;
    while (j + 1 < njobs && table[(j + 1) * 5 + 4] <= (long)blockIdx.x) ++j;
    job_s = j;
  }
  __syncthreads();
  const long* e = table + job_s * 5;
  const float* src = reinterpret_cast<const float*>(e[0]);
  unsigned char* dst = reinterpret_cast<unsigned char*>(e[1]);
  const int N = (int)e[2], K = (int)e[3], Npad = (N + 127) & ~127;
  const int tile = (int)(blockIdx.x - e[4]);
  const int rg = Npad / 64, kt = tile / rg, n = (tile % rg) * 64 + (threadIdx.x >> 2);
  const int cp = threadIdx.x & 3, c = cp ^ swz_w(n);
  unsigned h[4] = {0, 0, 0, 0}, m[4] = {0, 0, 0, 0}, l[4] = {0, 0, 0, 0};
  if (n < N) {
    const float* s = src + (long)n * K + 32 * kt + 4 * c;
    const float4 x0 = ld4(s), x1 = (32 * kt + 16 < K) ? ld4(s + 16) : make_float4(0.f, 0.f, 0.f, 0.f);
    split3_pair(x0.x, x0.y, h[0], m[0], l[0]);
    split3_pair(x0.z, x0.w, h[1], m[1], l[1]);
    split3_pair(x1.x, x1.y, h[2], m[2], l[2]);
    split3_pair(x1.z, x1.w, h[3], m[3], l[3]);
  }
  const long ps = (long)Npad * 64;
  unsigned char* d = dst + ((long)(kt * 3) * Npad + n) * 64 + cp * 16;
  *reinterpret_cast<uint4*>(d) = make_uint4(h[0], h[1], h[2], h[3]);
  *reinterpret_cast<uint4*>(d + ps) = make_uint4(m[0], m[1], m[2], m[3]);
  *reinterpret_cast<uint4*>(d + 2 * ps) = make_uint4(l[0], l[1], l[2], l[3]);
}

template <int TN, int AMODE>
__global__ __launch_bounds__(256, AMODE == MX_BNBWD ? 2 : 3) void gemm_nt_split3_kernel(GemmArgs g) {
  constexpr int BM = 128, BN = 16 * TN;
  constexpr int W_PLANE = BN * 64, STAGE = 3 * W_PLANE;
  constexpr int WPIECES = 3 * BN / 16, WPW = (WPIECES + 3) / 4;
  static_assert(4 * 2 * BN * 4 <= 2 * STAGE, "statistics staging does not fit");
  __shared__ __attribute__((aligned(1024))) unsigned char smem[2 * STAGE];
  const int tid = threadIdx.x, lane = tid & 63;
  const int wave = __builtin_amdgcn_readfirstlane(tid >> 6);
  const int l15 = lane & 15, q = lane >> 4;
  int tile_m = blockIdx.x, tile_n = blockIdx.y;
  if (g.xcd_nt > 0) {
    const int per_chunk = 8 * ((g.mt + 7) / 8) * g.xcd_nt;
    const int chunk = blockIdx.x / per_chunk, L = blockIdx.x % per_chunk, xcd = L & 7, j = L >> 3;
    tile_n = chunk * g.xcd_nt + j % g.xcd_nt;
    tile_m = (j / g.xcd_nt) * 8 + xcd;
    if (tile_m >= g.mt || tile_n >= g.zt) return;
  }
  const int m0 = tile_m * BM, n0 = tile_n * BN;
  const long zb = blockIdx.z;
  const float* A = g.a.p + zb * g.sa;
  const unsigned char* WP = reinterpret_cast<const unsigned char*>(g.b.p);
  float* C = g.c + zb * g.sc;
  const int nk = (g.K + 31) >> 5;
  const bool ktail = (g.K & 31) != 0;
  const long npad64 = (long)g.ldb * 64;

  const float* ap[2];
#pragma unroll
  for (int i = 0; i < 2; ++i) {
    const int gr = min(m0 + 32 * wave + 16 * i + l15, g.M - 1);
    ap[i] = A + (long)gr * g.lda + 4 * q;
  }
  const unsigned char* wsrc[WPW];
  int wdst[WPW];
#pragma unroll
  for (int i = 0; i < WPW; ++i) {
    const int pw = wave + 4 * i, p = pw / (BN / 16), rp = pw % (BN / 16);
    wsrc[i] = WP + ((long)p * g.ldb + n0 + 16 * rp) * 64 + lane * 16;
    wdst[i] = p * W_PLANE + rp * 1024;
  }
  auto issue_w = [&](int kt) {
    unsigned char* st = smem + (kt & 1) * STAGE;
#pragma unroll
    for (int i = 0; i < WPW; ++i)
      if (WPIECES % 4 == 0 || wave + 4 * i < WPIECES) glds16(wsrc[i] + 3 * npad64 * kt, st + wdst[i]);
  };
  f32x4 raw[2][2];
  f32x4 rawx[(AMODE == MX_BNBWD || AMODE == MX_BNACT) ? 2 : 1][2], cf[AMODE == MX_BNBWD ? 3 : AMODE == MX_BNACT ? 2 : 1][2];
  const long xoff = AMODE == MX_BNBWD ? (g.a.rowp + zb * g.sa) - A : 0;
  const float* gp[AMODE == MX_BNACT ? 2 : 1];
  if (AMODE == MX_BNACT) {
#pragma unroll
    for (int i = 0; i < 2; ++i) {
      const int gr = min(m0 + 32 * wave + 16 * i + l15, g.M - 1);
      gp[AMODE == MX_BNACT ? i : 0] = g.a.rowp + (long)(gr / g.a.rps) * g.K + 4 * q;
    }
  }
  auto load_a = [&](int kt) {
    const bool half = AMODE != MX_BNBWD && ktail && kt == nk - 1;
#pragma unroll
    for (int i = 0; i < 2; ++i) {
      raw[i][0] = *reinterpret_cast<const f32x4*>(ap[i] + 32 * kt);
      raw[i][1] = half ? f32x4{0.f, 0.f, 0.f, 0.f} : *reinterpret_cast<const f32x4*>(ap[i] + 32 * kt + 16);
      if (AMODE == MX_BNBWD) {
        rawx[AMODE == MX_BNBWD ? i : 0][0] = *reinterpret_cast<const f32x4*>(ap[i] + xoff + 32 * kt);
        rawx[AMODE == MX_BNBWD ? i : 0][1] = *reinterpret_cast<const f32x4*>(ap[i] + xoff + 32 * kt + 16);
      }
      if (AMODE == MX_BNACT) {
        rawx[AMODE == MX_BNACT ? i : 0][0] = *reinterpret_cast<const f32x4*>(gp[AMODE == MX_BNACT ? i : 0] + 32 * kt);
        rawx[AMODE == MX_BNACT ? i : 0][1] = *reinterpret_cast<const f32x4*>(gp[AMODE == MX_BNACT ? i : 0] + 32 * kt + 16);
      }
    }
    if (AMODE == MX_BNACT) {
      cf[0][0] = *reinterpret_cast<const f32x4*>(g.a.c1 + 32 * kt + 4 * q);
      cf[0][1] = *reinterpret_cast<const f32x4*>(g.a.c1 + 32 * kt + 4 * q + 16);
      cf[AMODE == MX_BNACT ? 1 : 0][0] = *reinterpret_cast<const f32x4*>(g.a.c2 + 32 * kt + 4 * q);
      cf[AMODE == MX_BNACT ? 1 : 0][1] = *reinterpret_cast<const f32x4*>(g.a.c2 + 32 * kt + 4 * q + 16);
    }
    if (AMODE == MX_BNBWD) {
#pragma unroll
      for (int c = 0; c < 3; ++c) {
        cf[AMODE == MX_BNBWD ? c : 0][0] = *reinterpret_cast<const f32x4*>(g.a.c1 + (long)c * g.K + 32 * kt + 4 * q);
        cf[AMODE == MX_BNBWD ? c : 0][1] = *reinterpret_cast<const f32x4*>(g.a.c1 + (long)c * g.K + 32 * kt + 4 * q + 16);
      }
    }
  };

  f32x4 acc[2][TN];
#pragma unroll
  for (int i = 0; i < 2; ++i)
#pragma unroll
    for (int j = 0; j < TN; ++j) acc[i][j] = f32x4{0.f, 0.f, 0.f, 0.f};
  const int woff = l15 * 64 + ((q ^ swz_w(l15)) << 4);

  MX_GEMM_STAMP(g, 0);
  issue_w(0);
  load_a(0);
  MX_GEMM_STAMP(g, 1);
  for (int kt = 0; kt < nk; ++kt) {
    asm volatile("s_waitcnt vmcnt(0)" ::: "memory");
    bf16x8 af[2][3];
#pragma unroll
    for (int i = 0; i < 2; ++i) {
      if (AMODE == MX_BNBWD) {
#pragma unroll
        for (int u = 0; u < 2; ++u)
#pragma unroll
          for (int e = 0; e < 4; ++e)
            raw[i][u][e] = cf[0][u][e] * raw[i][u][e] + (cf[AMODE == MX_BNBWD ? 1 : 0][u][e] * rawx[AMODE == MX_BNBWD ? i : 0][u][e] +
                                                         cf[AMODE == MX_BNBWD ? 2 : 0][u][e]);
      }
      if (AMODE == MX_BNACT) {
#pragma unroll
        for (int u = 0; u < 2; ++u)
#pragma unroll
          for (int e = 0; e < 4; ++e)
            raw[i][u][e] = swishf_(cf[0][u][e] * raw[i][u][e] + cf[AMODE == MX_BNACT ? 1 : 0][u][e]) * rawx[AMODE == MX_BNACT ? i : 0][u][e];
      }
      unsigned h[4], m[4], l[4];
      split3_pair(raw[i][0][0], raw[i][0][1], h[0], m[0], l[0]);
      split3_pair(raw[i][0][2], raw[i][0][3], h[1], m[1], l[1]);
      split3_pair(raw[i][1][0], raw[i][1][1], h[2], m[2], l[2]);
      split3_pair(raw[i][1][2], raw[i][1][3], h[3], m[3], l[3]);
      typedef unsigned u32x4 __attribute__((ext_vector_type(4)));
      af[i][0] = __builtin_bit_cast(bf16x8, u32x4{h[0], h[1], h[2], h[3]});
      af[i][1] = __builtin_bit_cast(bf16x8, u32x4{m[0], m[1], m[2], m[3]});
      af[i][2] = __builtin_bit_cast(bf16x8, u32x4{l[0], l[1], l[2], l[3]});
    }
    asm volatile("" ::: "memory");
    __builtin_amdgcn_s_barrier();
    asm volatile("" ::: "memory");
    if (kt + 1 < nk) { issue_w(kt + 1); load_a(kt + 1); }
    const unsigned char* st = smem + (kt & 1) * STAGE;
    constexpr int PW[6] = {0, 2, 1, 0, 1, 0}, PX[6] = {2, 0, 1, 1, 0, 0};
#pragma unroll
    for (int j = 0; j < TN; ++j) {
      bf16x8 wf[3];
#pragma unroll
      for (int p = 0; p < 3; ++p) wf[p] = *reinterpret_cast<const bf16x8*>(st + woff + p * W_PLANE + j * 1024);
#pragma unroll
      for (int t = 0; t < 6; ++t)
#pragma unroll
        for (int i = 0; i < 2; ++i)
          acc[i][j] = __builtin_amdgcn_mfma_f32_16x16x32_bf16(wf[PW[t]], af[i][PX[t]], acc[i][j], 0, 0, 0);
    }
  }
  MX_GEMM_STAMP(g, 2);
  __syncthreads();
  nt_epilogue<4, 1, 2, TN>(g, C, tile_m, m0, n0, acc, reinterpret_cast<float*>(smem), tid);
  MX_GEMM_STAMP(g, 3);
}

static int g_gemm_mode = getenv("MX_GEMM_SPLIT") ? atoi(getenv("MX_GEMM_SPLIT")) : 1;
static bool nt_uses_split(int N, int K) {
  return g_gemm_mode == 2 || (g_gemm_mode == 1 && K >= 128 && N >= 96 && (double)N / (64.0 * cdiv(N, 64)) >= 0.74);
}

template <int NJ>
static void launch_nt_split_t(const GemmArgs& g, int batch, hipStream_t st) {
  constexpr int BN = 64 * NJ;
  const int mt = cdiv(g.M, 128), nt = cdiv(g.N, BN);
  GemmArgs a = g;
  a.mt = mt;
  a.xcd_nt = 0;
  dim3 grid(mt, nt, batch);
  if (nt >= 2 && nt <= 16 && mt >= 64) { a.xcd_nt = nt; grid = dim3(8 * cdiv(mt, 8) * nt, 1, batch); }
  switch (g.a.mode) {
    case MX_PLAIN: hipLaunchKernelGGL((gemm_nt_split_kernel<MX_PLAIN, NJ>), grid, dim3(256), 0, st, a); break;
    case MX_BNACT: hipLaunchKernelGGL((gemm_nt_split_kernel<MX_BNACT, NJ>), grid, dim3(256), 0, st, a); break;
    default: hipLaunchKernelGGL((gemm_nt_split_kernel<MX_AFFINE, NJ>), grid, dim3(256), 0, st, a); break;
  }
}

static int g_split_nj = getenv("MX_GEMM_SPLIT_NJ") ? atoi(getenv("MX_GEMM_SPLIT_NJ")) : 0;
static void launch_nt_split(const GemmArgs& g, int batch, hipStream_t st) {
  const int forced = g_split_nj;
  auto score = [&](int bn, double eff) {
    const long nt = cdiv(g.N, bn), tiles = (long)cdiv(g.M, 128) * nt * batch;
    const double pad = (double)g.N / (double)(nt * bn);
    const double rounds = (double)tiles / 768.0;
    const double balance = rounds / (double)(long)(rounds + 0.999999);
    return eff * pad * balance;
  };
  auto cost = [&](int bn, double eff) {
    const double rounds = (double)cdiv(g.M, 128) * cdiv(g.N, bn) * batch / 768.0;
    const double full = (double)(long)rounds, tail = rounds - full;
    return (full + (tail > 0 ? (tail + 0.12 < 1.0 ? tail + 0.12 : 1.0) : 0.0)) * bn / eff;
  };
  const bool narrow = forced ? forced == 1
                    : g.K >= 1024 ? cost(64, 0.87) < cost(128, 1.0)
                                  : score(64, 0.92) > score(128, 1.0) + 1e-9;
  if (forced == 4) launch_nt_split_t<4>(g, batch, st);
  else if (narrow) launch_nt_split_t<1>(g, batch, st);
  else launch_nt_split_t<2>(g, batch, st);
}

static int g_split3_xcd_chunk = 6;
template <int TN>
static void launch_nt_split3_t(const GemmArgs& g, int batch, hipStream_t st) {
  constexpr int BN = 16 * TN;
  const int mt = cdiv(g.M, 128), nt = cdiv(g.N, BN);
  GemmArgs a = g;
  a.mt = mt;
  a.xcd_nt = 0;
  dim3 grid(mt, nt, batch);
  if (nt >= 2 && mt >= 64) {
    const int chunks = nt <= 16 ? 1 : cdiv(nt, g_split3_xcd_chunk);
    a.xcd_nt = cdiv(nt, chunks); a.zt = nt;
    grid = dim3(chunks * 8 * cdiv(mt, 8) * a.xcd_nt, 1, batch);
  }
  if (g.a.mode == MX_BNBWD) hipLaunchKernelGGL((gemm_nt_split3_kernel<TN, MX_BNBWD>), grid, dim3(256), 0, st, a);
  else if (g.a.mode == MX_BNACT) {
    if constexpr (TN <= 6) hipLaunchKernelGGL((gemm_nt_split3_kernel<TN, MX_BNACT>), grid, dim3(256), 0, st, a);
  } else hipLaunchKernelGGL((gemm_nt_split3_kernel<TN, MX_PLAIN>), grid, dim3(256), 0, st, a);
}

static void launch_nt_split3(const GemmArgs& g, int batch, hipStream_t st) {
  auto cost = [&](int bn, double eff) {
    const double per_cu = (double)cdiv(g.M, 128) * cdiv(g.N, bn) * batch / 256.0;
    return (per_cu + 0.5) * bn / eff;
  };
  const long wide_tiles = (long)cdiv(g.M, 128) * cdiv(g.N, 128) * batch;
  int bn = 128;
  if (g_split_nj >= 16) bn = g_split_nj;
  else if (g_split_nj == 1 || (g_split_nj != 2 && wide_tiles <= 300)) bn = 64;
  else if (g_split_nj != 2) {
    const bool shortk = g.K <= 512;
    const double e64 = shortk ? 0.90 : 0.85, e80 = shortk ? 0.97 : 0.90, e96 = shortk ? 1.03 : 0.94, e112 = 0.97;
    double best = cost(128, 1.0);
    if (cost(64, e64) < best) { best = cost(64, e64); bn = 64; }
    if (g_split_nj != 3) {
      if (g.N % 112 == 0 && cost(112, e112) < best) { best = cost(112, e112); bn = 112; }
      if (g.N % 96 == 0 && cost(96, e96) < best) { best = cost(96, e96); bn = 96; }
      if (g.N % 80 == 0 && cost(80, e80) < best) { best = cost(80, e80); bn = 80; }
    }
  }
  if (g.a.mode == MX_BNACT && bn > 96) bn = (g.N % 96 == 0) ? 96 : 64;
  switch (bn) {
    case 64: launch_nt_split3_t<4>(g, batch, st); break;
    case 80: launch_nt_split3_t<5>(g, batch, st); break;
    case 96: launch_nt_split3_t<6>(g, batch, st); break;
    case 112: launch_nt_split3_t<7>(g, batch, st); break;
    default: launch_nt_split3_t<8>(g, batch, st); break;
  }
}

struct NtCfg { int bm, bn; };
static const NtCfg kNtCfgs[] = {{128, 128}, {128, 96}, {128, 64}, {128, 48}, {128, 80}, {128, 32}, {128, 160}};
constexpr int kNumNtCfgs = sizeof(kNtCfgs) / sizeof(kNtCfgs[0]);

template <int WM, int WN, int TM, int TN>
static void launch_nt(const GemmArgs& g, int batch, hipStream_t st) {
  constexpr int BM = WM * TM * 16, BN = WN * TN * 16;
  const int mt = cdiv(g.M, BM), nt = cdiv(g.N, BN);
  GemmArgs a = g;
  a.mt = mt;
  a.xcd_nt = 0;
  dim3 grid(mt, nt, batch);
  if (nt >= 2 && nt <= 16 && mt >= 64) { a.xcd_nt = nt; grid = dim3(8 * cdiv(mt, 8) * nt, 1, batch); }
  switch (g.a.mode) {
    case MX_PLAIN: hipLaunchKernelGGL((gemm_nt_kernel<WM, WN, TM, TN, MX_PLAIN>), grid, dim3(256), 0, st, a); break;
    case MX_BNACT: hipLaunchKernelGGL((gemm_nt_kernel<WM, WN, TM, TN, MX_BNACT>), grid, dim3(256), 0, st, a); break;
    case MX_BNBWD: hipLaunchKernelGGL((gemm_nt_kernel<WM, WN, TM, TN, MX_BNBWD>), grid, dim3(256), 0, st, a); break;
    default: hipLaunchKernelGGL((gemm_nt_kernel<WM, WN, TM, TN, MX_AFFINE>), grid, dim3(256), 0, st, a); break;
  }
}

static int pick_nt_cfg(int M, int N) {
  int best = 0;
  double best_score = -1.0;
  for (int c = 0; c < kNumNtCfgs; ++c) {
    const NtCfg t = kNtCfgs[c];
    const long nt = cdiv(N, t.bn), tiles = (long)cdiv(M, t.bm) * nt;
    const double pad = (double)N / (double)(nt * t.bn);
    const double per_cu = (double)tiles / 256.0;
    const double balance = per_cu / (double)(long)(per_cu + 0.999999);
    double eff = t.bn >= 128 ? 1.0 : t.bn >= 96 ? 0.98 : t.bn >= 64 ? 0.95 : t.bn >= 48 ? 0.92 : 0.88;
    double score = eff * pad * balance;
    if (per_cu < 2.0) score *= 0.85;
    if (score > best_score + 1e-9) { best_score = score; best = c; }
  }
  return best;
}

static void dispatch_nt(const GemmArgs& g, int batch, hipStream_t st) {
  if (g.a.mode != MX_BNBWD && nt_uses_split(g.N, g.K)) {
    launch_nt_split(g, batch, st);
    return;
  }
  switch (pick_nt_cfg(g.M, g.N)) {
    case 0: launch_nt<2, 2, 4, 4>(g, batch, st); break;
    case 1: launch_nt<2, 2, 4, 3>(g, batch, st); break;
    case 2: launch_nt<2, 2, 4, 2>(g, batch, st); break;
    case 3: launch_nt<4, 1, 2, 3>(g, batch, st); break;
    case 4: launch_nt<4, 1, 2, 5>(g, batch, st); break;
    case 5: launch_nt<4, 1, 2, 2>(g, batch, st); break;
    default: launch_nt<2, 2, 4, 5>(g, batch, st); break;
  }
}

static int check_operand(const MxOperand& o, const char* nm) {
  MX_CHECK_ARG(o.p != nullptr, "gemm: operand %s is null", nm);
  MX_CHECK_ARG(((uintptr_t)o.p & 15) == 0, "gemm: operand %s not 16-byte aligned", nm);
  MX_CHECK_ARG(o.mode >= 0 && o.mode <= 3, "gemm: operand %s bad mode %d", nm, o.mode);
  if (o.mode != MX_PLAIN) {
    MX_CHECK_ARG(o.c1 && o.c2, "gemm: operand %s needs scale/shift", nm);
    MX_CHECK_ARG(o.rps > 0, "gemm: operand %s rows_per_sample must be > 0", nm);
  }
  return MX_OK;
}

static int tn_splits(int M, int N, int K, int* ksplit) {
  const TileCfg tc = kCfgs[pick_cfg(L_TN, M, N, K)];
  long tiles = (long)cdiv(M, tc.bm) * cdiv(N, tc.bn);
  constexpr long SPLIT_TARGET = 2048;
  int splits = (int)((SPLIT_TARGET + tiles - 1) / tiles);
  int maxs = cdiv(K, 512);
  if (splits > maxs) splits = maxs;
  if (splits < 1) splits = 1;
  int ks = cdiv(cdiv(K, splits), 32) * 32;
  *ksplit = ks;
  return cdiv(K, ks);
}

static int gemm_common(int layout, GemmArgs& g, int batch, hipStream_t st) {
  if (int e = check_operand(g.a, "A")) return e;
  if (int e = check_operand(g.b, "B")) return e;
  MX_CHECK_ARG(g.c != nullptr, "gemm: C is null");
  MX_CHECK_ARG(g.M > 0 && g.N > 0 && g.K > 0, "gemm: bad extents M=%d N=%d K=%d", g.M, g.N, g.K);
  MX_CHECK_ARG(g.lda % 4 == 0 && g.ldb % 4 == 0, "gemm: leading dims must be multiples of 4 (lda=%d ldb=%d)", g.lda, g.ldb);
  MX_CHECK_ARG(batch >= 1, "gemm: batch must be >= 1");
  g.stamps = mx_gemm_stamps;
  if (layout == L_NT) {
    MX_CHECK_ARG(g.K % 4 == 0, "gemm NT: K=%d must be a multiple of 4", g.K);
    if (g.b.mode == MX_PLAIN) dispatch_nt(g, batch, st);
    else dispatch<L_NT>(g, batch, st);
  } else if (layout == L_NN) {
    MX_CHECK_ARG(g.K % 4 == 0 && g.N % 4 == 0, "gemm NN: K=%d and N=%d must be multiples of 4", g.K, g.N);
    dispatch<L_NN>(g, batch, st);
  } else {
    MX_CHECK_ARG(g.M % 4 == 0 && g.N % 4 == 0, "gemm TN: M=%d and N=%d must be multiples of 4", g.M, g.N);
    MX_CHECK_ARG(batch == 1, "gemm TN: not batched");
    const int splits = tn_splits(g.M, g.N, g.K, &g.ksplit);
    if (splits > 1) {
      float* dW = g.c;
      g.c = g.ws; g.sc = (long)g.M * g.N; g.ldc = g.N;
      hipMemsetAsync(g.ws, 0, sizeof(float) * (size_t)splits * g.M * g.N, st);
      dispatch<L_TN>(g, splits, st);
      MX_LAUNCH_CHECK();
      mx_launch_parts_reduce(g.ws, splits, g.M * g.N, dW, st);
    } else {
      dispatch<L_TN>(g, 1, st);
    }
  }
  MX_LAUNCH_CHECK();
  return MX_OK;
}

__global__ __launch_bounds__(256) void transpose_kernel(const float* __restrict__ src, float* __restrict__ dst, int rows, int cols) {
  __shared__ float t[32][33];
  const int bx = blockIdx.x * 32, by = blockIdx.y * 32;
  const int tx = threadIdx.x & 31, ty = threadIdx.x >> 5;
#pragma unroll
  for (int i = 0; i < 32; i += 8) {
    const int r = by + ty + i, c = bx + tx;
    if (r < rows && c < cols) t[ty + i][tx] = src[(long)r * cols + c];
  }
  __syncthreads();
#pragma unroll
  for (int i = 0; i < 32; i += 8) {
    const int c = bx + ty + i, r = by + tx;
    if (r < rows && c < cols) dst[(long)c * rows + r] = t[tx][ty + i];
  }
}

__global__ __launch_bounds__(256) void transpose_batch_kernel(const long* __restrict__ table, int n) {
  __shared__ float t[32][33];
  __shared__ int job;
  if (threadIdx.x == 0) {
    int j = 0;
    while (j + 1 < n && table[(j + 1) * 5 + 4] <= (long)blockIdx.x) ++j;
    job = j;
  }
  __syncthreads();
  const long* e = table + job * 5;
  const float* src = reinterpret_cast<const float*>(e[0]);
  float* dst = reinterpret_cast<float*>(e[1]);
  const int rows = (int)e[2], cols = (int)e[3];
  const int tile = (int)(blockIdx.x - e[4]), tx_n = (cols + 31) / 32;
  const int bx = (tile % tx_n) * 32, by = (tile / tx_n) * 32;
  const int tx = threadIdx.x & 31, ty = threadIdx.x >> 5;
#pragma unroll
  for (int i = 0; i < 32; i += 8) {
    const int r = by + ty + i, c = bx + tx;
    if (r < rows && c < cols) t[ty + i][tx] = src[(long)r * cols + c];
  }
  __syncthreads();
#pragma unroll
  for (int i = 0; i < 32; i += 8) {
    const int c = bx + ty + i, r = by + tx;
    if (r < rows && c < cols) dst[(long)c * rows + r] = t[tx][ty + i];
  }
}

extern "C" {

int mx_transpose_batch(const long* table, int n, int total_tiles, void* stream) {
  MX_CHECK_ARG(table && n > 0 && total_tiles > 0, "transpose_batch: bad arguments");
  hipLaunchKernelGGL(transpose_batch_kernel, dim3(total_tiles), dim3(256), 0, (hipStream_t)stream, table, n);
  MX_LAUNCH_CHECK();
  return MX_OK;
}

int mx_transpose(const float* src, float* dst, int rows, int cols, void* stream) {
  MX_CHECK_ARG(src && dst && rows > 0 && cols > 0, "transpose: bad arguments");
  hipLaunchKernelGGL(transpose_kernel, dim3(cdiv(cols, 32), cdiv(rows, 32)), dim3(256), 0, (hipStream_t)stream, src, dst, rows, cols);
  MX_LAUNCH_CHECK();
  return MX_OK;
}

long mx_pw_planes_bytes(int N, int K) {
  if (N <= 0 || K <= 0 || K % 16) return MX_EARG;
  return (long)((N + 127) & ~127) * ((K + 31) & ~31) * 6;
}

int mx_pw_planes_tiles(int N, int K) {
  if (N <= 0 || K <= 0 || K % 16) return MX_EARG;
  return (((N + 127) & ~127) / 64) * ((K + 31) / 32);
}

int mx_pw_planes_batch(const long* table, int n, int total_tiles, void* stream) {
  MX_CHECK_ARG(table && n > 0 && total_tiles > 0, "pw_planes_batch: bad arguments");
  hipLaunchKernelGGL(split_planes_kernel, dim3(total_tiles), dim3(256), 0, (hipStream_t)stream, table, n);
  MX_LAUNCH_CHECK();
  return MX_OK;
}

int mx_pw_fwd_uses_planes(int M, int K, int N) {
  if (M <= 0 || K % 16) return 0;
  if (K % 32) return (g_gemm_mode != 0 && K >= 48 && N >= 96) ? 1 : 0;
  if (nt_uses_split(N, K)) return 1;
  return (g_gemm_mode == 1 && K >= 192 && N >= 48) ? 1 : 0;
}

int mx_pw_fwd_planes(const float* A, const void* Wplanes, float* C, int M, int K, int N, int lda, int ldc,
                     const float* bias, const float* residual, int relu, float* stats, void* stream) {
  MX_CHECK_ARG(A && Wplanes && C, "pw_fwd_planes: null pointer");
  MX_CHECK_ARG(M > 0 && N > 0 && K > 0 && K % 16 == 0, "pw_fwd_planes: bad extents M=%d N=%d K=%d (K must be a multiple of 16)", M, N, K);
  MX_CHECK_ARG(lda % 4 == 0 && lda >= K && ldc >= N, "pw_fwd_planes: bad leading dimensions lda=%d ldc=%d", lda, ldc);
  MX_CHECK_ARG((((uintptr_t)A | (uintptr_t)Wplanes | (uintptr_t)C) & 15) == 0, "pw_fwd_planes: pointers must be 16-byte aligned");
  GemmArgs g{};
  g.a = MxOperand{A, nullptr, nullptr, nullptr, MX_PLAIN, 1};
  g.b = MxOperand{reinterpret_cast<const float*>(Wplanes), nullptr, nullptr, nullptr, MX_PLAIN, 1};
  g.c = C; g.M = M; g.N = N; g.K = K; g.lda = lda; g.ldb = (N + 127) & ~127; g.ldc = ldc;
  g.bias = bias; g.residual = residual; g.relu = relu; g.stats = stats;
  g.stamps = mx_gemm_stamps;
  launch_nt_split3(g, 1, (hipStream_t)stream);
  MX_LAUNCH_CHECK();
  return MX_OK;
}

int mx_pw_fwd_act_uses_planes(int M, int K, int N) {
  return (g_gemm_mode != 0 && M >= 65536 && K % 32 == 0 && K >= 192 && N >= 48 && N <= 128) ? 1 : 0;
}

int mx_pw_fwd_planes_act(const float* A, const float* scale, const float* shift, const float* gate, int rows_per_sample,
                         const void* Wplanes, float* C, int M, int K, int N, int lda, int ldc, float* stats, void* stream) {
  MX_CHECK_ARG(A && scale && shift && gate && Wplanes && C, "pw_fwd_planes_act: null pointer");
  MX_CHECK_ARG(M > 0 && N > 0 && K > 0 && K % 32 == 0 && rows_per_sample > 0, "pw_fwd_planes_act: bad extents M=%d N=%d K=%d rows_per_sample=%d", M, N, K, rows_per_sample);
  MX_CHECK_ARG(lda % 4 == 0 && lda >= K && ldc >= N, "pw_fwd_planes_act: bad leading dimensions lda=%d ldc=%d", lda, ldc);
  MX_CHECK_ARG((((uintptr_t)A | (uintptr_t)scale | (uintptr_t)shift | (uintptr_t)gate | (uintptr_t)Wplanes | (uintptr_t)C) & 15) == 0,
               "pw_fwd_planes_act: pointers must be 16-byte aligned");
  GemmArgs g{};
  g.a = MxOperand{A, scale, shift, gate, MX_BNACT, rows_per_sample};
  g.b = MxOperand{reinterpret_cast<const float*>(Wplanes), nullptr, nullptr, nullptr, MX_PLAIN, 1};
  g.c = C; g.M = M; g.N = N; g.K = K; g.lda = lda; g.ldb = (N + 127) & ~127; g.ldc = ldc;
  g.stats = stats;
  launch_nt_split3(g, 1, (hipStream_t)stream);
  MX_LAUNCH_CHECK();
  return MX_OK;
}

int mx_pw_dgrad_bnbwd_planes(const float* G, const float* X, const float* coef, const void* WtPlanes, float* dX, int M, int K, int N,
                             int ldg, int ldx, const float* residual, void* stream) {
  MX_CHECK_ARG(G && X && coef && WtPlanes && dX, "pw_dgrad_bnbwd_planes: null pointer");
  MX_CHECK_ARG(M > 0 && N > 0 && K > 0 && K % 32 == 0, "pw_dgrad_bnbwd_planes: bad extents M=%d N=%d K=%d (K must be a multiple of 32)", M, N, K);
  MX_CHECK_ARG(ldg % 4 == 0 && ldg >= K && ldx >= N, "pw_dgrad_bnbwd_planes: bad leading dimensions");
  MX_CHECK_ARG((((uintptr_t)G | (uintptr_t)X | (uintptr_t)coef | (uintptr_t)WtPlanes | (uintptr_t)dX) & 15) == 0, "pw_dgrad_bnbwd_planes: pointers must be 16-byte aligned");
  GemmArgs g{};
  g.a = MxOperand{G, coef, coef + K, X, MX_BNBWD, 1};
  g.b = MxOperand{reinterpret_cast<const float*>(WtPlanes), nullptr, nullptr, nullptr, MX_PLAIN, 1};
  g.c = dX; g.M = M; g.N = N; g.K = K; g.lda = ldg; g.ldb = (N + 127) & ~127; g.ldc = ldx;
  g.residual = residual;
  launch_nt_split3(g, 1, (hipStream_t)stream);
  MX_LAUNCH_CHECK();
  return MX_OK;
}

int mx_set_gemm_mode(int mode) {
  MX_CHECK_ARG(mode >= 0 && mode <= 2, "set_gemm_mode: mode %d (0 fp32 MFMA, 1 split for MFMA-bound shapes, 2 split everywhere)", mode);
  g_gemm_mode = mode;
  return MX_OK;
}

int mx_get_gemm_mode(void) { return g_gemm_mode; }

bool mx_wgrad_uses_split(int R, int Co, int Ci);

int mx_gemm_uses_split(int kind, int M, int N, int K) {
  if (kind == 0) return nt_uses_split(N, K) ? 1 : 0;
  return mx_wgrad_uses_split(K, M, N) ? 1 : 0;
}

int mx_pw_fwd_parts(int M, int N, int K) {
  if (M <= 0 || N <= 0 || K <= 0) return MX_EARG;
  return cdiv(M, 128);
}


int mx_pw_fwd(const float* A, int a_mode, const float* a_scale, const float* a_shift, const float* a_gate,
              int rows_per_sample, const float* W, float* C, int M, int K, int N, int lda, int ldc,
              const float* bias, const float* residual, int relu, float* stats, void* stream) {
  GemmArgs g{};
  g.a = MxOperand{A, a_scale, a_shift, a_gate, a_mode, rows_per_sample};
  g.b = MxOperand{W, nullptr, nullptr, nullptr, MX_PLAIN, 1};
  g.c = C; g.M = M; g.N = N; g.K = K; g.lda = lda; g.ldb = K; g.ldc = ldc;
  g.bias = bias; g.residual = residual; g.relu = relu; g.stats = stats;
  return gemm_common(L_NT, g, 1, (hipStream_t)stream);
}

int mx_pw_dgrad(const float* G, const float* W, float* dX, int M, int K, int N, int ldg, int ldx,
                const float* residual, void* stream) {
  GemmArgs g{};
  g.a = MxOperand{G, nullptr, nullptr, nullptr, MX_PLAIN, 1};
  g.b = MxOperand{W, nullptr, nullptr, nullptr, MX_PLAIN, 1};
  g.c = dX; g.M = M; g.N = N; g.K = K; g.lda = ldg; g.ldb = N; g.ldc = ldx;
  g.residual = residual;
  return gemm_common(L_NN, g, 1, (hipStream_t)stream);
}

int mx_pw_dgrad_bnbwd(const float* G, const float* X, const float* coef, const float* Wt, float* dX, float* dZ, int M, int K, int N,
                      int ldg, int ldx, const float* residual, void* stream) {
  MX_CHECK_ARG(G && X && coef && Wt && dX && dZ, "pw_dgrad_bnbwd: null pointer");
  MX_CHECK_ARG(dZ != G && dZ != X, "pw_dgrad_bnbwd: dZ must not alias G or X (other N tiles still read them)");
  MX_CHECK_ARG((((uintptr_t)X | (uintptr_t)dZ | (uintptr_t)coef) & 15) == 0 && K % 4 == 0, "pw_dgrad_bnbwd: alignment");
  GemmArgs g{};
  g.a = MxOperand{G, coef, coef + K, X, MX_BNBWD, 1};
  g.b = MxOperand{Wt, nullptr, nullptr, nullptr, MX_PLAIN, 1};
  g.c = dX; g.M = M; g.N = N; g.K = K; g.lda = ldg; g.ldb = K; g.ldc = ldx;
  g.residual = residual;
  g.a_out = dZ;
  return gemm_common(L_NT, g, 1, (hipStream_t)stream);
}

long mx_pw_wgrad_ws(int R, int Co, int Ci) {
  if (R <= 0 || Co <= 0 || Ci <= 0 || Co % 4 || Ci % 4) return MX_EARG;
  int ks;
  const int splits = tn_splits(Co, Ci, R, &ks);
  return splits > 1 ? (long)splits * Co * Ci * 4 : 0;
}

int mx_pw_wgrad(const float* G, const float* X, int x_mode, const float* x_scale, const float* x_shift,
                const float* x_gate, int rows_per_sample, float* dW, int R, int Co, int Ci, int ldg, int ldx,
                void* ws, long ws_bytes, void* stream) {
  const long need = mx_pw_wgrad_ws(R, Co, Ci);
  MX_CHECK_ARG(need >= 0, "pw_wgrad: bad extents R=%d Co=%d Ci=%d", R, Co, Ci);
  MX_CHECK_ARG(need == 0 || (ws && ws_bytes >= need && ((uintptr_t)ws & 15) == 0), "pw_wgrad: %ld bytes of scratch required (mx_pw_wgrad_ws)", need);
  GemmArgs g{};
  g.a = MxOperand{G, nullptr, nullptr, nullptr, MX_PLAIN, 1};
  g.b = MxOperand{X, x_scale, x_shift, x_gate, x_mode, rows_per_sample};
  g.c = dW; g.M = Co; g.N = Ci; g.K = R; g.lda = ldg; g.ldb = ldx; g.ldc = Ci;
  g.ws = (float*)ws;
  return gemm_common(L_TN, g, 1, (hipStream_t)stream);
}

int mx_bgemm(int layout, const float* A, const float* B, float* C, int M, int N, int K, int lda, int ldb, int ldc,
             long sa, long sb, long sc, int batch, int relu, void* stream) {
  MX_CHECK_ARG(layout == L_NT || layout == L_NN, "bgemm: layout must be 0 (NT) or 1 (NN)");
  GemmArgs g{};
  g.a = MxOperand{A, nullptr, nullptr, nullptr, MX_PLAIN, 1};
  g.b = MxOperand{B, nullptr, nullptr, nullptr, MX_PLAIN, 1};
  g.c = C; g.M = M; g.N = N; g.K = K; g.lda = lda; g.ldb = ldb; g.ldc = ldc;
  g.sa = sa; g.sb = sb; g.sc = sc; g.relu = relu;
  return gemm_common(layout, g, batch, (hipStream_t)stream);
}

}
```

### muscle_amd/engine.py

```python
from __future__ import annotations

import os

from dataclasses import dataclass, field
from typing import Dict, List, Optional

import torch

from . import ops
from .arch import BlockCfg, NetCfg
from .ops import BNState


@dataclass
class BlockTape:
    cfg: BlockCfg
    H: int
    W: int
    Ho: int
    Wo: int
    x: torch.Tensor
    x_st: Optional[BNState]
    e_raw: Optional[torch.Tensor] = None
    bn0: Optional[BNState] = None
# ... 133 lines not shown
    plan = getattr(backbone, "_wt_plan", None)
    views = [v for _, v in ws]
    if plan is None or not plan.matches(views):
        if plan is not None:
            backbone.__dict__.setdefault("_wt_plans_retired", []).append(plan)
        plan = None if torch.cuda.is_current_stream_capturing() else ops.WeightPlan(views)
        backbone._wt_plan = plan
    if plan is not None and ops.get_gemm_mode() != 0:
        for (w, _), im in zip(ws, plan.run_forward()):
            if im is not None:
                tape.wp[id(w)] = im
    if not backward:
        return
    side = _WgradLane(dev).s
    if side is not None:
        side.wait_stream(torch.cuda.current_stream())
    with torch.cuda.stream(side):
        if plan is not None:
            wts, ims = plan.run_backward()
            for (w, _), wt, im in zip(ws, wts, ims):
                tape.wt[id(w)] = wt
                if im is not None and ops.get_gemm_mode() != 0:
                    tape.wtp[id(w)] = im
        elif side is not None:
            for w, v in ws:
                tape.wt[id(w)] = ops.transpose(v)
        if side is not None:
            tape.wt_event = side.record_event()


def backbone_forward(backbone, cfg: NetCfg, img: torch.Tensor, training: bool,
                     drop_u: Optional[Dict[int, torch.Tensor]] = None, save: bool = True) -> Tape:
    N, _, H, W = img.shape
    dev = img.device
    tape = Tape(training=training, N=N)
    lo, hi = cfg.stem_pad
    H0, W0 = (H + lo + hi - 3) // 2 + 1, (W + lo + hi - 3) // 2 + 1
    tape.H0, tape.W0 = H0, W0
    if save or training or not EVAL_FOLD:
        _prepare_weights(backbone, cfg, tape, dev, backward=save)
    tape.cols = ops.stem_im2col(img, H0, W0, lo)
    C0 = cfg.stem_out
    raw, stats = ops.pw_fwd(tape.cols, stem_weight28(backbone), C0, want_stats=True) if training else \
        (ops.pw_fwd(tape.cols, stem_weight28(backbone), C0), None)
    tape.stem_raw = raw.view(N, H0, W0, C0)
    tape.stem_bn = ops.bn_finalize(stats, N * H0 * W0, backbone._bn0, training)

    drop_scales: Dict[int, torch.Tensor] = {}
    if training and drop_u is None:
        idx = [b.index for b in cfg.blocks if b.skip and b.drop_rate]
        if idx:
            rates = tuple(1.0 - cfg.blocks[i].drop_rate for i in idx)
            key = (rates, str(dev))
            if key not in _keep_cache:
                _keep_cache[key] = torch.tensor(rates, dtype=torch.float32).to(dev).view(-1, 1)
            keep = _keep_cache[key]
            rs = torch.floor(keep + torch.rand(len(idx), N, device=dev)) / keep
            drop_scales = {i: rs[j] for j, i in enumerate(idx)}
    x, x_st, h, w = tape.stem_raw, tape.stem_bn, H0, W0
    fold = None
    if not training and not save and EVAL_FOLD:
        fold = getattr(backbone, "_eval_fold", None)
        if fold is not None and fold["fingerprint"] != fold_fingerprint(backbone, cfg):
            fold = backbone._eval_fold = fold_eval_bn(backbone, cfg)
        elif fold is None:
            fold = fold_eval_bn(backbone, cfg)
    for b in cfg.blocks:
        m = _blk(backbone, b.index)
        ho, wo = b.out_size(h), b.out_size(w)
        t = BlockTape(cfg=b, H=h, W=w, Ho=ho, Wo=wo, x=x, x_st=x_st)
        if fold is not None:
            t.out = _block_forward_eval(m, b, fold[b.index], (fold["one"], fold["zero"]), x, x_st, N, h, w, ho, wo)
            t.x = None
            tape.blocks.append(t)
            if b.index == 0:
                tape.cols = tape.stem_raw = None
            if len(tape.blocks) >= 2 and tape.blocks[-2].cfg.index not in cfg.taps:
                tape.blocks[-2].out = None
            x, x_st, h, w = t.out, None, ho, wo
            continue
        M, Mo = N * h * w, N * ho * wo
        if b.expand:
            assert x_st is None
            st0 = None
            t.e_raw = ops.pw_fwd(x.view(M, b.cin), m._expand_conv.weight.view(b.cexp, b.cin), b.cexp, want_stats=training,
                                 planes=tape.wp.get(id(m._expand_conv.weight)))
            if training:
                t.e_raw, st0 = t.e_raw
            t.e_raw = t.e_raw.view(N, h, w, b.cexp)
            t.bn0 = ops.bn_finalize(st0, M, m._bn0, training)
            dw_in, dw_st = t.e_raw, t.bn0
        else:
            dw_in, dw_st = x, x_st
        st1 = None
        t.d_raw = ops.dwconv_fwd(dw_in, m._depthwise_conv.weight, b.kernel, b.stride, b.pad_lo, ho, wo, st=dw_st,
                                 want_stats=training)
        if training:
            t.d_raw, st1 = t.d_raw
        t.bn1 = ops.bn_finalize(st1, Mo, m._bn1, training)
        d2 = t.d_raw.view(Mo, b.cexp)
        pooled = ops.pool_sum(d2, ho * wo, st=t.bn1, act=True)
        t.s, t.h, t.gate = ops.se_fwd(pooled, 1.0 / (ho * wo), m._se_reduce.weight.view(b.se, b.cexp), m._se_reduce.bias,
                                      m._se_expand.weight.view(b.cexp, b.se), m._se_expand.bias)
        st2 = None
        if b.cout > MATERIALISE_ABOVE:
            t.a = ops.bn_apply(d2, t.bn1, gate=t.gate, rows_per_sample=ho * wo, act=True)
            t.p_raw = ops.pw_fwd(t.a, m._project_conv.weight.view(b.cout, b.cexp), b.cout, want_stats=training,
                                 planes=tape.wp.get(id(m._project_conv.weight)))
        else:
            t.p_raw = ops.pw_fwd(d2, m._project_conv.weight.view(b.cout, b.cexp), b.cout, a_mode=ops.BNACT,
                                 a_scale=t.bn1.scale, a_shift=t.bn1.shift, a_gate=t.gate, rows_per_sample=ho * wo,
                                 want_stats=training, planes=tape.wp.get(id(m._project_conv.weight)))
        if training:
            t.p_raw, st2 = t.p_raw
        t.bn2 = ops.bn_finalize(st2, Mo, m._bn2, training)
        if b.skip and training and b.drop_rate:
            if drop_u is not None:
                keep = 1.0 - b.drop_rate
                t.row_scale = torch.floor(keep + drop_u[b.index].to(dev, torch.float32)) / keep
            else:
                t.row_scale = drop_scales[b.index]
        res = None
        if b.skip:
            assert x_st is None
            res = x.view(M, b.cin)
        t.out = ops.bn_apply(t.p_raw, t.bn2, row_scale=t.row_scale, residual=res, rows_per_sample=ho * wo).view(N, ho, wo, b.cout)
        tape.blocks.append(t)
        x, x_st, h, w = t.out, None, ho, wo
        if not save:
            t.x = t.e_raw = t.d_raw = t.p_raw = t.a = None
            if b.index == 0:
                tape.cols = tape.stem_raw = None
            if len(tape.blocks) >= 2 and tape.blocks[-2].cfg.index not in cfg.taps:
                tape.blocks[-2].out = None
    ops.flush_batch_counters()
    return tape


class GradSink:

    def __init__(self):
        self.bufs: Dict[int, torch.Tensor] = {}

    def of(self, p: torch.nn.Parameter) -> torch.Tensor:
        g = self.bufs.get(id(p))
        if g is None:
            g = torch.zeros_like(p, memory_format=torch.contiguous_format)
            self.bufs[id(p)] = g
        return g


FOLD_BN0_EARLY = os.environ.get("MUSCLE_FOLD_BN0_EARLY", "1") == "1"
DW_S2_FUSED = os.environ.get("MUSCLE_DW_S2_FUSED", "1") == "1"
WGRAD_SIDE_STREAM = os.environ.get("MUSCLE_WGRAD_STREAM", "1") == "1"
_side_streams: Dict[int, "torch.cuda.Stream"] = {}


class _WgradLane:
    def __init__(self, device):
        self.s = None
        self.pending = []
        self.keep = []
        if WGRAD_SIDE_STREAM:
            key = device.index if device.index is not None else torch.cuda.current_device()
            if key not in _side_streams:
                _side_streams[key] = torch.cuda.Stream(device=device)
            self.s = _side_streams[key]

    def _queue(self, launch, *reads):
        if self.s is None:
            return launch()
        self.pending.append((launch, reads))

    def wgrad(self, G, X, dW, **kw):
        return self._queue(lambda: ops.pw_wgrad(G, X, dW, **kw), G, X)

    def wgrad_bnbwd(self, G, G2, coef, X, dW):
        return self._queue(lambda: ops.pw_wgrad_bnbwd(G, G2, coef, X, dW), G, X, G2, coef)

    def dw_reduce(self, scratch, dW):
        return self._queue(lambda: ops.dw_parts_reduce(scratch, dW), scratch)

    def flush(self):
        if self.s is None or not self.pending:
            return
        self.s.wait_stream(torch.cuda.current_stream())
        with torch.cuda.stream(self.s):
            for launch, _ in self.pending:
                launch()
        self.keep.extend(reads for _, reads in self.pending)
        self.pending = []

    def progress(self, done, module):
        if self.s is None:
            return done(module)
        self.flush()
        self.s.wait_stream(torch.cuda.current_stream())
        with torch.cuda.stream(self.s):
            done(module)

    def join(self):
        self.flush()
        if self.s is not None:
            torch.cuda.current_stream().wait_stream(self.s)
        self.keep = []


def _dw_input(t: BlockTape):
    return (t.e_raw, t.bn0) if t.cfg.expand else (t.x, t.x_st)


def _project_backward(lane, tape: Tape, t: BlockTape, m, g_out, sink: GradSink):
    b, hw = t.cfg, t.Ho * t.Wo
    Mo = tape.N * hw
    dp = ops.bn_backward(g_out.reshape(Mo, b.cout), t.p_raw, m._bn2, t.bn2, sink.of(m._bn2.weight), sink.of(m._bn2.bias), tape.training,
                         row_scale=t.row_scale, rows_per_sample=hw)
    if t.a is not None:
        lane.wgrad(dp, t.a, sink.of(m._project_conv.weight).view(b.cout, b.cexp))
        t.a = None
    else:
        lane.wgrad(dp, t.d_raw.view(Mo, b.cexp), sink.of(m._project_conv.weight).view(b.cout, b.cexp), x_mode=ops.BNACT,
                   x_scale=t.bn1.scale, x_shift=t.bn1.shift, x_gate=t.gate, rows_per_sample=hw)
    ga = ops.pw_dgrad(dp, m._project_conv.weight.view(b.cout, b.cexp), b.cexp, wt=tape.wt.get(id(m._project_conv.weight)),
                      planes=tape.wtp.get(id(m._project_conv.weight)))
    lane.flush()
    return ga


def _se_bn1_coeffs(tape: Tape, t: BlockTape, m, ga, sink: GradSink):
    b, hw = t.cfg, t.Ho * t.Wo
    Mo = tape.N * hw
    pooled5 = ops.se_bn1_pool(ga, t.d_raw.view(Mo, b.cexp), t.bn1, hw)
    gh = ops.se_bwd(pooled5[0], t.gate, t.s, t.h, m._se_expand.weight.view(b.cexp, b.se),
                    sink.of(m._se_reduce.weight).view(b.se, b.cexp), sink.of(m._se_reduce.bias),
                    sink.of(m._se_expand.weight).view(b.cexp, b.se), sink.of(m._se_expand.bias))
    return ops.bn1_coeffs(pooled5, t.gate, gh, m._se_reduce.weight.view(b.se, b.cexp), 1.0 / hw, Mo, m._bn1, t.bn1,
                          sink.of(m._bn1.weight), sink.of(m._bn1.bias), tape.training)


def _depthwise_backward(lane, tape: Tape, t: BlockTape, m, ga, c1, add, skip_res, sink: GradSink):
    b, N = t.cfg, tape.N
    dw_in, dw_st = _dw_input(t)
    res = None if dw_st is not None else skip_res
    if b.stride == 1 and b.pad_lo == (b.kernel - 1) // 2:
        return ops.dwconv_bwd_fused(ga.view(N, t.Ho, t.Wo, b.cexp), t.d_raw, t.gate, add, t.bn1, c1, dw_in, dw_st,
                                    m._depthwise_conv.weight, sink.of(m._depthwise_conv.weight), b.kernel, b.pad_lo,
                                    residual=res, defer=lane.dw_reduce)
    if DW_S2_FUSED and b.stride == 2 and dw_st is not None:
        return ops.dwconv_bwd_fused_s2(ga.view(N, t.Ho, t.Wo, b.cexp), t.d_raw, t.gate, add, t.bn1, c1, dw_in, dw_st,
                                       m._depthwise_conv.weight, sink.of(m._depthwise_conv.weight), b.kernel, b.pad_lo,
                                       defer=lane.dw_reduce)
    dd = ops.bn_backward_from_coeffs(ga, t.d_raw.view(N * t.Ho * t.Wo, b.cexp), t.bn1, c1, gate=t.gate, gate_add=add,
                                     rows_per_sample=t.Ho * t.Wo, out=ga).view(N, t.Ho, t.Wo, b.cexp)
    ops.dwconv_bwd_weight(dw_in, dd, sink.of(m._depthwise_conv.weight), b.kernel, b.stride, b.pad_lo, st=dw_st)
    return ops.dwconv_bwd_data(dd, m._depthwise_conv.weight, b.kernel, b.stride, b.pad_lo, t.H, t.W, residual=res), None


def _bn0_expand_backward(lane, backbone, cfg: NetCfg, tape: Tape, t: BlockTape, m, gx, part0, skip_res, sink: GradSink):
    b, N, training = t.cfg, tape.N, tape.training
    dw_in, dw_st = _dw_input(t)
    bn_mod = m._bn0 if b.expand else backbone._bn0
    M = N * t.H * t.W
    raw2, gx2 = dw_in.view(M, dw_in.shape[3]), gx.view(M, dw_in.shape[3])
    res = skip_res.reshape(M, b.cin) if skip_res is not None else None
    if part0 is not None:
        c0 = ops.bn_bwd_coeffs(part0, M, bn_mod, dw_st, sink.of(bn_mod.weight), sink.of(bn_mod.bias), training)
        wtp = tape.wtp.get(id(m._expand_conv.weight)) if b.expand else None
        if FOLD_BN0_EARLY and b.stride == 1 and wtp is not None and ops.bnbwd_fold_takes(M, b.cexp, b.cin) == "small":
            lane.wgrad_bnbwd(gx2, raw2, c0, t.x.view(M, b.cin), sink.of(m._expand_conv.weight).view(b.cexp, b.cin))
            g_in = ops.pw_dgrad_bnbwd_planes(gx2, raw2, c0, wtp, b.cin, residual=res)
            lane.flush()
            return g_in.view(N, t.H, t.W, b.cin)
        dz = ops.bn_bwd_apply_plain(gx2, raw2, c0, gx2)
    else:
        dz = ops.bn_backward(gx2, raw2, bn_mod, dw_st, sink.of(bn_mod.weight), sink.of(bn_mod.bias), training, act=dw_st, out=gx2)
    if not b.expand:
        dw28 = torch.zeros(cfg.stem_out, 28, dtype=torch.float32, device=dz.device)
        ops.pw_wgrad(dz, tape.cols, dw28)
        sink.of(backbone._conv_stem.weight).view(cfg.stem_out, 27).add_(dw28[:, :27])
        return None
    lane.wgrad(dz, t.x.view(M, b.cin), sink.of(m._expand_conv.weight).view(b.cexp, b.cin))
    g_in = ops.pw_dgrad(dz, m._expand_conv.weight.view(b.cexp, b.cin), b.cin, wt=tape.wt.get(id(m._expand_conv.weight)),
                        planes=tape.wtp.get(id(m._expand_conv.weight)), residual=res)
    lane.flush()
    return g_in.view(N, t.H, t.W, b.cin)


def backbone_backward(backbone, cfg: NetCfg, tape: Tape, tap_grads: Dict[int, torch.Tensor], sink: GradSink):
    g_out: Optional[torch.Tensor] = None
    lane = _WgradLane(tape.blocks[0].out.device)
    if tape.wt_event is not None:
        torch.cuda.current_stream().wait_event(tape.wt_event)
    done = getattr(sink, "block_done", None) if getattr(sink, "on_ready", None) is not None else None
    for t in reversed(tape.blocks):
        m = _blk(backbone, t.cfg.index)
        tg = tap_grads.get(t.cfg.index)
        if tg is not None:
            g_out = tg if g_out is None else g_out + tg
        if g_out is None:
            continue
        ga = _project_backward(lane, tape, t, m, g_out, sink)
        c1, add = _se_bn1_coeffs(tape, t, m, ga, sink)
        skip_res = g_out if t.cfg.skip else None
        gx, part0 = _depthwise_backward(lane, tape, t, m, ga, c1, add, skip_res, sink)
        del ga
        if _dw_input(t)[1] is not None:
            g_out = _bn0_expand_backward(lane, backbone, cfg, tape, t, m, gx, part0, skip_res, sink)
        else:
            g_out = gx
        if done is not None:
            lane.progress(done, m)
    lane.join()
```

### muscle_amd/ops.py

```python
from __future__ import annotations

import os
from typing import NamedTuple, Optional

import torch

from ._lib import call, lib, ptr, stream

PLAIN, BNACT, AFFINE = 0, 1, 2


class BNState(NamedTuple):
    scale: torch.Tensor
    shift: torch.Tensor
    mean: torch.Tensor
    rstd: torch.Tensor


def _f32(*shape, device):
    return torch.empty(shape, dtype=torch.float32, device=device)


_scratch_bufs: dict = {}
_wgrad_ws: dict = {}
# ... 30 lines not shown
    try:
        call(name, *args)
    except Exception:
        key = (torch.cuda.current_device(), stream())
        buf = _scratch_bufs.get(key)
        if buf is not None:
            buf[:65536].zero_()
        raise


def _per_mode(ask):
    memo: dict = {}

    def cached(*shape):
        key = (get_gemm_mode(), *shape)
        if key not in memo:
            memo[key] = ask(*shape)
        return memo[key]
    return cached


@_per_mode
def _planes_take(M, K, N_out):
    return bool(lib().mx_pw_fwd_uses_planes(M, K, N_out))


@_per_mode
def _planes_act_take(M, K, N_out):
    return bool(lib().mx_pw_fwd_act_uses_planes(M, K, N_out))


def pw_fwd(A, W, N_out, *, a_mode=PLAIN, a_scale=None, a_shift=None, a_gate=None, rows_per_sample=1,
           bias=None, residual=None, relu=False, want_stats=False, out=None, ldc=None, planes=None):
    M, K = A.shape
    ldc = ldc or N_out
    if out is None:
        out = _f32(M, ldc, device=A.device)
    stats = None
    if want_stats:
        stats = _f32(lib().mx_pw_fwd_parts(M, N_out, K), 2, N_out, device=A.device)
    if planes is not None and a_mode == PLAIN and _planes_take(M, K, N_out):
        call("mx_pw_fwd_planes", ptr(A), planes, ptr(out), M, K, N_out, A.stride(0), ldc, ptr(bias), ptr(residual), int(relu),
             ptr(stats), stream())
    elif (planes is not None and a_mode == BNACT and a_gate is not None and bias is None and residual is None and not relu
          and _planes_act_take(M, K, N_out)):
        call("mx_pw_fwd_planes_act", ptr(A), ptr(a_scale), ptr(a_shift), ptr(a_gate), rows_per_sample, planes, ptr(out), M, K, N_out,
             A.stride(0), ldc, ptr(stats), stream())
    else:
        call("mx_pw_fwd", ptr(A), a_mode, ptr(a_scale), ptr(a_shift), ptr(a_gate), rows_per_sample, ptr(W), ptr(out),
             M, K, N_out, A.stride(0), ldc, ptr(bias), ptr(residual), int(relu), ptr(stats), stream())
    return (out, stats) if want_stats else out


def set_gemm_mode(mode: int):
    call("mx_set_gemm_mode", int(mode))


def get_gemm_mode() -> int:
    return int(lib().mx_get_gemm_mode())


def set_wgrad_kernel(kernel: int = -1, groups: int = -1):
    call("mx_set_wgrad_kernel", int(kernel), int(groups))


def get_wgrad_kernel() -> int:
    return int(lib().mx_get_wgrad_kernel())


class TransposePlan:

    def __init__(self, weights):
        dev = weights[0].device
        self.key = tuple((w.data_ptr(), tuple(w.shape)) for w in weights)
        self.dst = [_f32(w.shape[1], w.shape[0], device=dev) for w in weights]
        rows, tile = [], 0
        for w, d in zip(weights, self.dst):
            r, c = w.shape
            rows.append([w.data_ptr(), d.data_ptr(), r, c, tile])
            tile += ((r + 31) // 32) * ((c + 31) // 32)
        self.n, self.tiles = len(rows), tile
        self.table = torch.tensor(rows, dtype=torch.int64).to(dev)
        torch.cuda.current_stream(dev).synchronize()

    def matches(self, weights):
        return len(weights) == self.n and all(k[0] == w.data_ptr() and k[1] == tuple(w.shape) for k, w in zip(self.key, weights))

    def run(self):
        call("mx_transpose_batch", ptr(self.table), self.n, self.tiles, stream())
        return self.dst


class PlanesPlan:

    def __init__(self, mats):
        dev = mats[0].device
        L = lib()
        rows, tile, off = [], 0, 0
        sizes = []
        for m in mats:
            n, k = m.shape
            nb = L.mx_pw_planes_bytes(n, k) if m.is_contiguous() else -1
            sizes.append(nb)
            if nb > 0:
                off += (nb + 1023) & ~1023
        self.buf = torch.empty(max(off, 1024), dtype=torch.uint8, device=dev)
        base, off = self.buf.data_ptr(), 0
        self.images = []
        for m, nb in zip(mats, sizes):
            if nb <= 0:
                self.images.append(None)
                continue
            n, k = m.shape
            rows.append([m.data_ptr(), base + off, n, k, tile])
            self.images.append(base + off)
            tile += L.mx_pw_planes_tiles(n, k)
            off += (nb + 1023) & ~1023
        self.n, self.tiles = len(rows), tile
        self.table = torch.tensor(rows, dtype=torch.int64).to(dev) if rows else None
        torch.cuda.current_stream(dev).synchronize()

    def run(self):
        if self.n:
            call("mx_pw_planes_batch", ptr(self.table), self.n, self.tiles, stream())
        return self.images


class WeightPlan:

    def __init__(self, weights):
        self.t = TransposePlan(weights)
        self.key = self.t.key
        self.fwd = PlanesPlan(weights)
        self.bwd = PlanesPlan(self.t.dst)

    def matches(self, weights):
        return self.t.matches(weights)

    def run_forward(self):
        return self.fwd.run()

    def run_backward(self):
        wt = self.t.run()
        return wt, self.bwd.run()


def transpose(W):
    rows, cols = W.shape
    out = _f32(cols, rows, device=W.device)
    call("mx_transpose", ptr(W), ptr(out), rows, cols, stream())
    return out


def pw_dgrad(G, W, N_in, *, residual=None, out=None, wt=None, planes=None):
    M, K = G.shape
    if out is None:
        out = _f32(M, N_in, device=G.device)
    if K % 4 == 0:
        if planes is not None and _planes_take(M, K, N_in):
            call("mx_pw_fwd_planes", ptr(G), planes, ptr(out), M, K, N_in, G.stride(0), N_in, None, ptr(residual), 0, None, stream())
            return out
        call("mx_pw_fwd", ptr(G), PLAIN, None, None, None, 1, ptr(wt if wt is not None else transpose(W)), ptr(out), M, K, N_in, G.stride(0), N_in,
             None, ptr(residual), 0, None, stream())
        return out
    call("mx_pw_dgrad", ptr(G), ptr(W), ptr(out), M, K, N_in, G.stride(0), N_in, ptr(residual), stream())
    return out


def pw_dgrad_bnbwd(G, X, coef, W, N_in, *, residual=None, wt=None):
    M, K = G.shape
    out = _f32(M, N_in, device=G.device)
    dz = torch.empty_like(G)
    call("mx_pw_dgrad_bnbwd", ptr(G), ptr(X), ptr(coef), ptr(wt if wt is not None else transpose(W)), ptr(out), ptr(dz), M, K, N_in,
         G.stride(0), N_in, ptr(residual), stream())
    return out, dz


def pw_dgrad_bnbwd_planes(G, X, coef, planes, N_in, *, residual=None):
    M, K = G.shape
    out = _f32(M, N_in, device=G.device)
    call("mx_pw_dgrad_bnbwd_planes", ptr(G), ptr(X), ptr(coef), planes, ptr(out), M, K, N_in, G.stride(0), N_in, ptr(residual), stream())
    return out


@_per_mode
def bnbwd_fold_takes(M, K, N):
    if not _planes_take(M, K, N):
        return None
    if lib().mx_pw_wgrad_small_bnbwd_ok(M, K, N):
        return "small"
    if lib().mx_pw_wgrad_small_ws(M, K, N, PLAIN) <= 0 and lib().mx_pw_wgrad_tile_bnbwd_ok(M, K, N):
        return "tile"
    return None


def pw_wgrad_bnbwd(G, G2, coef, X, dW):
    R, Co = G.shape
    Ci = X.shape[1]
    if lib().mx_pw_wgrad_small_bnbwd_ok(R, Co, Ci):
        need = lib().mx_pw_wgrad_small_ws(R, Co, Ci, PLAIN)
        ws = _wgrad_workspace(G.device, max(need, 16))
        call("mx_pw_wgrad_small_bnbwd", ptr(G), ptr(G2), ptr(coef), ptr(X), ptr(dW), R, Co, Ci, G.stride(0), X.stride(0), ws.data_ptr(), ws.numel(), stream())
        return
    need = lib().mx_pw_wgrad_tile_ws(R, Co, Ci, PLAIN)
    ws = _wgrad_workspace(G.device, max(need, 16))
    call("mx_pw_wgrad_tile_bnbwd", ptr(G), ptr(G2), ptr(coef), ptr(X), ptr(dW), R, Co, Ci, G.stride(0), X.stride(0), ws.data_ptr(), ws.numel(), stream())


def wgrad_bnbwd_dz_takes(R, Co, Ci) -> bool:
    return bool(lib().mx_pw_wgrad_tile_bnbwd_dz_ok(R, Co, Ci, Co, Ci))


def pw_wgrad_bnbwd_dz(G, G2, coef, X, dW, dz=None):
    R, Co = G.shape
    Ci = X.shape[1]
    if dz is None:
        dz = torch.empty_like(G)
    need = lib().mx_pw_wgrad_tile_ws(R, Co, Ci, PLAIN)
    ws = _wgrad_workspace(G.device, max(need, 16))
    call("mx_pw_wgrad_tile_bnbwd_dz", ptr(G), ptr(G2), ptr(coef), ptr(X), ptr(dW), ptr(dz), R, Co, Ci, G.stride(0), X.stride(0),
         ws.data_ptr(), ws.numel(), stream())
    return dz


WGRAD_TILE = os.environ.get("MUSCLE_WGRAD_TILE", "1") == "1"
WGRAD_SMALL = True


def pw_wgrad(G, X, dW, *, x_mode=PLAIN, x_scale=None, x_shift=None, x_gate=None, rows_per_sample=1):
    R, Co = G.shape
    Ci = X.shape[1]
    if WGRAD_SMALL and dW.is_contiguous():
        need = lib().mx_pw_wgrad_small_ws(R, Co, Ci, x_mode)
        if need > 0:
            ws = _wgrad_workspace(G.device, need)
            call("mx_pw_wgrad_small", ptr(G), ptr(X), x_mode, ptr(x_scale), ptr(x_shift), ptr(x_gate), rows_per_sample, ptr(dW),
                 R, Co, Ci, G.stride(0), X.stride(0), ws.data_ptr(), ws.numel(), stream())
            return
    if WGRAD_TILE and dW.is_contiguous():
        need = lib().mx_pw_wgrad_tile_ws(R, Co, Ci, x_mode)
        if need > 0:
            ws = _wgrad_workspace(G.device, need)
            call("mx_pw_wgrad_tile", ptr(G), ptr(X), x_mode, ptr(x_scale), ptr(x_shift), ptr(x_gate), rows_per_sample, ptr(dW),
                 R, Co, Ci, G.stride(0), X.stride(0), ws.data_ptr(), ws.numel(), stream())
            return
    need = lib().mx_pw_wgrad_ws(R, Co, Ci)
    ws = _wgrad_workspace(G.device, need) if need > 0 else None
    call("mx_pw_wgrad", ptr(G), ptr(X), x_mode, ptr(x_scale), ptr(x_shift), ptr(x_gate), rows_per_sample, ptr(dW),
         R, Co, Ci, G.stride(0), X.stride(0), ws.data_ptr() if ws is not None else None, ws.numel() if ws is not None else 0, stream())


def bgemm(layout, A, B, out, M, N, K, *, relu=False):
    b = A.shape[0]
    call("mx_bgemm", layout, ptr(A), ptr(B), ptr(out), M, N, K, A.stride(1), B.stride(1), out.stride(1),
         A.stride(0), B.stride(0), out.stride(0), b, int(relu), stream())
    return out


def colstats(X2d):
    rows, C = X2d.shape
    part = _f32(lib().mx_colreduce_parts(rows, C), 2, C, device=X2d.device)
    call("mx_colstats", ptr(X2d), rows, C, ptr(part), stream())
    return part


def bn_finalize(stats, count, bn: torch.nn.BatchNorm2d, training: bool) -> BNState:
    C = bn.num_features
    dev = bn.weight.device
    buf = _f32(4, C, device=dev)
    b0, b1, b2, b3 = buf.unbind(0)
    base = buf.data_ptr()
    mom = 0.0 if bn.momentum is None else float(bn.momentum)
    call("mx_bn_finalize", ptr(stats), stats.shape[0] if stats is not None else 0, C, float(count), ptr(bn.weight), ptr(bn.bias), ptr(bn.running_mean),
         ptr(bn.running_var), mom, float(bn.eps), int(training), base, base + 4 * C, base + 8 * C, base + 12 * C,
         _acc_scratch(dev, 128 * C) if training else None, stream())
    if training:
        _nbt_pending.append(bn.num_batches_tracked)
    return BNState(b0, b1, b2, b3)


def fold_block(We, bn0, bn1, Wp, bn2, out=None):
    dev = Wp.device
    cout, cexp = Wp.shape
    cin = We.shape[1] if We is not None else cexp
    if out is not None:
        f, vec = out, out["_vec"]
    else:
        f = {}
        vec = f["_vec"] = _f32(3, cexp, device=dev)
        if We is not None:
            f["We"], f["be"] = _f32(cexp, cin, device=dev), vec[0]
        f["bn1"] = BNState(vec[1], vec[2], None, None)
        f["Wp"], f["bp"] = _f32(cout, cexp, device=dev), _f32(cout, device=dev)

    def four(bn):
        return (ptr(bn.weight), ptr(bn.bias), ptr(bn.running_mean), ptr(bn.running_var), float(bn.eps))
    none4 = (None, None, None, None, 0.0)
    call("mx_fold_block", ptr(We.detach()) if We is not None else None, *(four(bn0) if We is not None else none4), *four(bn1),
         ptr(Wp.detach()), *four(bn2), cin, cexp, cout, ptr(f.get("We")), ptr(f.get("be")), ptr(vec[1]), ptr(vec[2]),
         ptr(f["Wp"]), ptr(f["bp"]), stream())
    return f


_nbt_pending: list = []


def flush_batch_counters():
    if _nbt_pending:
        torch._foreach_add_(_nbt_pending, 1)
        _nbt_pending.clear()


def bn_apply(P2d, st: BNState, *, row_scale=None, residual=None, gate=None, rows_per_sample=1, act=False, out=None):
    rows, C = P2d.shape
    if out is None:
        out = torch.empty_like(P2d)
    call("mx_bn_apply", ptr(P2d), ptr(st.scale), ptr(st.shift), ptr(row_scale), ptr(residual), ptr(gate), ptr(out), rows, C,
         rows_per_sample, int(act), stream())
    return out
# ... 383 lines not shown
```

Before: 339.4 images/sec.

## Fuse SE/BN1 five-way pooling into the project-conv dgrad GEMM epilogue

Adds a pool5 epilogue to the NT GEMM kernels. While writing the dgrad output, it computes the five per-sample SE/BN1 backward reductions (swish derivative terms against the stored pre-activation) and writes per-tile partials. A small join kernel then reduces those partials per sample. This removes a separate full read of the dgrad output and activation in se_bn1_pool for blocks with many rows and a modest expanded channel count. In exchange the epilogue does more work, occupancy hints drop for some tile shapes, and the request is passed through thread-local state.

```diff
diff --git a/include/muscle_hip.h b/include/muscle_hip.h
--- a/include/muscle_hip.h
+++ b/include/muscle_hip.h
@@ -27,6 +27,10 @@
 int mx_pw_fwd_uses_planes(int M, int K, int N);
 int mx_pw_fwd_planes(const float* A, const void* Wplanes, float* C, int M, int K, int N, int lda, int ldc,
                      const float* bias, const float* residual, int relu, float* stats, void* stream);
+
+long mx_pw_pool5_bytes(int planes, int M, int K, int N, int rows_per_sample);
+int mx_pw_epilogue_pool5(const float* X, const float* scale, const float* shift, int rows_per_sample, float* part5, long bytes);
+int mx_se_pool5_join(const float* part5, long rows, int C, int rows_per_sample, float* out5, void* stream);
 
 int mx_transpose(const float* src, float* dst, int rows, int cols, void* stream);
 int mx_transpose_batch(const long* table, int n, int total_tiles, void* stream);
diff --git a/muscle_amd/csrc/bn.hip b/muscle_amd/csrc/bn.hip
--- a/muscle_amd/csrc/bn.hip
+++ b/muscle_amd/csrc/bn.hip
@@ -321,6 +321,36 @@
   }
 }
 
+__global__ __launch_bounds__(256) void se_pool5_join_kernel(const float* __restrict__ part, int C, int rps, int nsamp, int R,
+                                                            float* __restrict__ out) {
+  __shared__ float4 sm[256];
+  const int tid = threadIdx.x;
+  const int tcols = 256 / R, tc = tid % tcols, tr = tid / tcols;
+  const int c4 = blockIdx.x * tcols + tc, k = blockIdx.y, n = blockIdx.z;
+  const bool in = 4 * c4 < C;
+  const long r0 = (long)n * rps;
+  const int t0 = (int)(r0 / 128), t1 = (int)((r0 + rps - 1) / 128);
+  float4 s = make_float4(0.f, 0.f, 0.f, 0.f);
+  if (in) {
+    const float* p = part + ((long)(t0 + n) * 5 + k) * C + 4 * c4;
+#pragma unroll 4
+    for (int t = t0 + tr; t <= t1; t += R) {
+      const float4 v = ld4(p + (long)(t - t0) * 5 * C);
+      s.x += v.x; s.y += v.y; s.z += v.z; s.w += v.w;
+    }
+  }
+  float* dst = out + ((long)k * nsamp + n) * C + 4 * c4;
+  if (R == 1) {
+    if (in) st4(dst, s);
+    return;
+  }
+  sm[tid] = s;
+  __syncthreads();
+  if (tr != 0 || !in) return;
+  for (int r = 1; r < R; ++r) { const float4 v = sm[tid + r * tcols]; s.x += v.x; s.y += v.y; s.z += v.z; s.w += v.w; }
+  st4(dst, s);
+}
+
 constexpr int BN_MAX_SLICES = 64;
 __global__ __launch_bounds__(256) void bn_parts_reduce_kernel(const float* part, int P, int C, int rows_per_slice, double* acc) {
   __shared__ double sh[2][8][32];
@@ -713,6 +743,19 @@
   return MX_OK;
 }
 
+int mx_se_pool5_join(const float* part5, long rows, int C, int rows_per_sample, float* out5, void* stream) {
+  MX_CHECK_ARG(part5 && out5 && rows > 0 && C > 0 && C % 4 == 0 && rows_per_sample >= 128 && rows % rows_per_sample == 0,
+               "se_pool5_join: bad args");
+  MX_CHECK_ARG((((uintptr_t)part5 | (uintptr_t)out5) & 15) == 0, "se_pool5_join: pointers must be 16-byte aligned");
+  const int N = (int)(rows / rows_per_sample);
+  const int tiles = (rows_per_sample + 127) / 128 + 1;
+  const int R = tiles <= 8 ? 1 : tiles <= 64 ? 4 : tiles <= 512 ? 16 : 64;
+  hipLaunchKernelGGL(se_pool5_join_kernel, dim3(cdiv(C / 4, 256 / R), 5, N), dim3(256), 0, (hipStream_t)stream, part5, C, rows_per_sample, N, R,
+                     out5);
+  MX_LAUNCH_CHECK();
+  return MX_OK;
+}
+
 int mx_bn1_sums_finalize(const float* pooled5, const float* gate, const float* gh, const float* W1, float inv_hw, float* add,
                          int N, int C, int SQ, double count, const float* gamma, const float* mean, const float* rstd, int training,
                          float* dgamma, float* dbeta, float* c1, float* c2, float* c3, void* stream) {
diff --git a/muscle_amd/csrc/gemm.hip b/muscle_amd/csrc/gemm.hip
--- a/muscle_amd/csrc/gemm.hip
+++ b/muscle_amd/csrc/gemm.hip
@@ -21,6 +21,11 @@
   unsigned long long* stamps;
   float* a_out;
   float* ws;
+  const float* pool_x;
+  const float* pool_a;
+  const float* pool_b;
+  float* pool_part;
+  int pool_rps;
 };
 
 #ifndef MX_GEMM_STAMP
@@ -353,8 +358,121 @@
 }
 
 template <int WM, int WN, int TM, int TN>
+static __device__ __forceinline__ void nt_epilogue_pool5(const GemmArgs& g, float* C, int tile_m, int m0, int n0, f32x4 (&acc)[TM][TN],
+                                                         float* red, int tid) {
+  constexpr int BM = WM * TM * 16, BN = WN * TN * 16;
+  const int lane = tid & 63, wave = tid >> 6;
+  const int l15 = lane & 15, q = lane >> 4;
+  const int wm = wave / WN, wn = wave % WN;
+  const int n_first = m0 / g.pool_rps;
+  const int bound = (n_first + 1) * g.pool_rps;
+  const int m_end = min(m0 + BM, g.M);
+  const bool straddle = bound < m_end;
+  const int colw = wn * TN * 16 + 4 * q;
+  const int row0 = m0 + wm * TM * 16 + l15;
+  const long istep = 16L * g.ldc;
+  const long xoff = g.pool_x - C;
+#define MX_POOL5_ONE(e, S)                                                          \
+  {                                                                                 \
+    const float xv = x[e], ga = v[e];                                               \
+    const float z = aa[e] * xv + bb[e], sg = sigmoidf_(z);                          \
+    const float act = z * sg, sp = sg * (1.f + z * (1.f - sg));                     \
+    S[0][e] += ga * act; S[1][e] += ga * sp; S[2][e] += sp;                         \
+    S[3][e] += ga * sp * xv; S[4][e] += sp * xv;                                    \
+  }
+  if (!straddle && m0 + BM <= g.M && n0 + BN <= g.N) {
+    const long idx0 = (long)row0 * g.ldc + n0 + colw;
+    float* cp[TM];
+#pragma unroll
+    for (int i = 0; i < TM; ++i) cp[i] = C + idx0 + i * istep;
+#pragma unroll
+    for (int j = 0; j < TN; ++j) {
+      const f32x4 aa = *reinterpret_cast<const f32x4*>(g.pool_a + n0 + colw + 16 * j);
+      const f32x4 bb = *reinterpret_cast<const f32x4*>(g.pool_b + n0 + colw + 16 * j);
+      f32x4 xr[TM];
+#pragma unroll
+      for (int i = 0; i < TM; ++i) xr[i] = *reinterpret_cast<const f32x4*>(cp[i] + xoff + 16 * j);
+      f32x4 s[5];
+#pragma unroll
+      for (int k = 0; k < 5; ++k) s[k] = f32x4{0.f, 0.f, 0.f, 0.f};
+#pragma unroll
+      for (int i = 0; i < TM; ++i) {
+        const f32x4 v = acc[i][j], x = xr[i];
+        __builtin_nontemporal_store(v, reinterpret_cast<f32x4*>(cp[i] + 16 * j));
+#pragma unroll
+        for (int e = 0; e < 4; ++e) MX_POOL5_ONE(e, s)
+      }
+#pragma unroll
+      for (int k = 0; k < 5; ++k) {
+#pragma unroll
+        for (int e = 0; e < 4; ++e) s[k][e] = row16_sum(s[k][e]);
+        if (l15 == 0) *reinterpret_cast<f32x4*>(red + (wm * 5 + k) * BN + colw + 16 * j) = s[k];
+      }
+    }
+  } else {
+    float* cp[TM];
+#pragma unroll
+    for (int i = 0; i < TM; ++i) cp[i] = C + (long)min(row0 + 16 * i, g.M - 1) * g.ldc;
+#pragma unroll
+    for (int j = 0; j < TN; ++j) {
+      const int col = n0 + colw + 16 * j;
+      const bool cok = col < g.N;
+      const int colc = cok ? col : 0;
+      const f32x4 aa = *reinterpret_cast<const f32x4*>(g.pool_a + colc);
+      const f32x4 bb = *reinterpret_cast<const f32x4*>(g.pool_b + colc);
+      f32x4 sa[5], sb[5];
+#pragma unroll
+      for (int k = 0; k < 5; ++k) sa[k] = sb[k] = f32x4{0.f, 0.f, 0.f, 0.f};
+#pragma unroll
+      for (int i = 0; i < TM; ++i) {
+        const int row = row0 + 16 * i;
+        const bool ok = row < g.M && cok;
+        const f32x4 v = acc[i][j], x = *reinterpret_cast<const f32x4*>(cp[i] + xoff + colc);
+        if (ok) __builtin_nontemporal_store(v, reinterpret_cast<f32x4*>(cp[i] + colc));
+        const float ma = (row < bound && ok) ? 1.f : 0.f, mb = (row >= bound && ok) ? 1.f : 0.f;
+#pragma unroll
+        for (int e = 0; e < 4; ++e) {
+          const float xv = x[e], ga = v[e];
+          const float z = aa[e] * xv + bb[e], sg = sigmoidf_(z);
+          const float act = z * sg, sp = sg * (1.f + z * (1.f - sg));
+          const float t0 = ga * act, t1 = ga * sp, t3 = ga * sp * xv, t4 = sp * xv;
+          sa[0][e] = fmaf(ma, t0, sa[0][e]); sb[0][e] = fmaf(mb, t0, sb[0][e]);
+          sa[1][e] = fmaf(ma, t1, sa[1][e]); sb[1][e] = fmaf(mb, t1, sb[1][e]);
+          sa[2][e] = fmaf(ma, sp, sa[2][e]); sb[2][e] = fmaf(mb, sp, sb[2][e]);
+          sa[3][e] = fmaf(ma, t3, sa[3][e]); sb[3][e] = fmaf(mb, t3, sb[3][e]);
+          sa[4][e] = fmaf(ma, t4, sa[4][e]); sb[4][e] = fmaf(mb, t4, sb[4][e]);
+        }
+      }
+#pragma unroll
+      for (int k = 0; k < 5; ++k) {
+#pragma unroll
+        for (int e = 0; e < 4; ++e) { sa[k][e] = row16_sum(sa[k][e]); sb[k][e] = row16_sum(sb[k][e]); }
+        if (l15 == 0) {
+          *reinterpret_cast<f32x4*>(red + (wm * 5 + k) * BN + colw + 16 * j) = sa[k];
+          *reinterpret_cast<f32x4*>(red + ((WM + wm) * 5 + k) * BN + colw + 16 * j) = sb[k];
+        }
+      }
+    }
+  }
+#undef MX_POOL5_ONE
+  __syncthreads();
+  const int nslot = straddle ? 2 : 1;
+  for (int i = tid; i < nslot * 5 * BN; i += 256) {
+    const int slot = i / (5 * BN), r = i - slot * 5 * BN, k = r / BN, col = r - k * BN;
+    float v = red[(slot * WM * 5 + k) * BN + col];
+#pragma unroll
+    for (int w = 1; w < WM; ++w) v += red[((slot * WM + w) * 5 + k) * BN + col];
+    if (n0 + col < g.N) g.pool_part[((long)(tile_m + n_first + slot) * 5 + k) * g.N + n0 + col] = v;
+  }
+}
+
+template <int WM, int WN, int TM, int TN, bool POOL = false>
 static __device__ __forceinline__ void nt_epilogue(const GemmArgs& g, float* C, int tile_m, int m0, int n0, f32x4 (&acc)[TM][TN],
                                                    float* smem, int tid) {
+  if constexpr (POOL) {
+    nt_epilogue_pool5<WM, WN, TM, TN>(g, C, tile_m, m0, n0, acc, smem, tid);
+    return;
+  }
   constexpr int BN = WN * TN * 16;
   const int lane = tid & 63, wave = tid >> 6;
   const int l15 = lane & 15, q = lane >> 4;
@@ -473,14 +591,16 @@
 }
 
 constexpr int gemm_nt_waves(int acc) { return acc <= 48 ? 4 : acc <= 64 ? 3 : 2; }
-
-template <int WM, int WN, int TM, int TN, int AMODE>
-__global__ __launch_bounds__(256, gemm_nt_waves(TM * TN * 4 + (AMODE == MX_BNBWD ? 16 : 0))) void gemm_nt_kernel(GemmArgs g) {
+constexpr int gemm_nt_pool_waves(int tm, int acc) { return tm > 2 && gemm_nt_waves(acc) > 2 ? gemm_nt_waves(acc) - 1 : gemm_nt_waves(acc); }
+
+template <int WM, int WN, int TM, int TN, int AMODE, bool POOL = false>
+__global__ __launch_bounds__(256, POOL ? gemm_nt_pool_waves(TM, TM * TN * 4) : gemm_nt_waves(TM * TN * 4 + (AMODE == MX_BNBWD ? 16 : 0))) void gemm_nt_kernel(GemmArgs g) {
   constexpr int BM = WM * TM * 16, BN = WN * TN * 16, LS = 20;
   constexpr int PA = (BM * 4 + 255) / 256, PB = (BN * 4 + 255) / 256;
   constexpr int SMEM = 2 * (BM + BN) * LS;
   static_assert(WM * WN == 4, "four waves");
   static_assert(WM * 2 * BN <= SMEM, "statistics staging does not fit the operand buffers");
+  static_assert(!POOL || (AMODE == MX_PLAIN && 2 * WM * 5 * BN <= SMEM), "pool5 staging does not fit the operand buffers");
   __shared__ __attribute__((aligned(16))) float smem[SMEM];
   const int tid = threadIdx.x, lane = tid & 63, wave = tid >> 6;
   const int l15 = lane & 15, q = lane >> 4;
@@ -597,7 +717,7 @@
     __syncthreads();
   }
   MX_GEMM_STAMP(g, 2);
-  nt_epilogue<WM, WN, TM, TN>(g, C, tile_m, m0, n0, acc, smem, tid);
+  nt_epilogue<WM, WN, TM, TN, POOL>(g, C, tile_m, m0, n0, acc, smem, tid);
   MX_GEMM_STAMP(g, 3);
 }
 
@@ -871,12 +991,13 @@
   *reinterpret_cast<uint4*>(d + 2 * ps) = make_uint4(l[0], l[1], l[2], l[3]);
 }
 
-template <int TN, int AMODE>
+template <int TN, int AMODE, bool POOL = false>
 __global__ __launch_bounds__(256, AMODE == MX_BNBWD ? 2 : 3) void gemm_nt_split3_kernel(GemmArgs g) {
   constexpr int BM = 128, BN = 16 * TN;
   constexpr int W_PLANE = BN * 64, STAGE = 3 * W_PLANE;
   constexpr int WPIECES = 3 * BN / 16, WPW = (WPIECES + 3) / 4;
   static_assert(4 * 2 * BN * 4 <= 2 * STAGE, "statistics staging does not fit");
+  static_assert(!POOL || (AMODE == MX_PLAIN && 2 * 4 * 5 * BN * 4 <= 2 * STAGE), "pool5 staging does not fit");
   __shared__ __attribute__((aligned(1024))) unsigned char smem[2 * STAGE];
   const int tid = threadIdx.x, lane = tid & 63;
   const int wave = __builtin_amdgcn_readfirstlane(tid >> 6);
@@ -1020,7 +1141,7 @@
   }
   MX_GEMM_STAMP(g, 2);
   __syncthreads();
-  nt_epilogue<4, 1, 2, TN>(g, C, tile_m, m0, n0, acc, reinterpret_cast<float*>(smem), tid);
+  nt_epilogue<4, 1, 2, TN, POOL>(g, C, tile_m, m0, n0, acc, reinterpret_cast<float*>(smem), tid);
   MX_GEMM_STAMP(g, 3);
 }
 
@@ -1085,7 +1206,8 @@
   if (g.a.mode == MX_BNBWD) hipLaunchKernelGGL((gemm_nt_split3_kernel<TN, MX_BNBWD>), grid, dim3(256), 0, st, a);
   else if (g.a.mode == MX_BNACT) {
     if constexpr (TN <= 6) hipLaunchKernelGGL((gemm_nt_split3_kernel<TN, MX_BNACT>), grid, dim3(256), 0, st, a);
-  } else hipLaunchKernelGGL((gemm_nt_split3_kernel<TN, MX_PLAIN>), grid, dim3(256), 0, st, a);
+  } else if (g.pool_x) hipLaunchKernelGGL((gemm_nt_split3_kernel<TN, MX_PLAIN, true>), grid, dim3(256), 0, st, a);
+  else hipLaunchKernelGGL((gemm_nt_split3_kernel<TN, MX_PLAIN>), grid, dim3(256), 0, st, a);
 }
 
 static void launch_nt_split3(const GemmArgs& g, int batch, hipStream_t st) {
@@ -1132,7 +1254,10 @@
   dim3 grid(mt, nt, batch);
   if (nt >= 2 && nt <= 16 && mt >= 64) { a.xcd_nt = nt; grid = dim3(8 * cdiv(mt, 8) * nt, 1, batch); }
   switch (g.a.mode) {
-    case MX_PLAIN: hipLaunchKernelGGL((gemm_nt_kernel<WM, WN, TM, TN, MX_PLAIN>), grid, dim3(256), 0, st, a); break;
+    case MX_PLAIN:
+      if (g.pool_x) hipLaunchKernelGGL((gemm_nt_kernel<WM, WN, TM, TN, MX_PLAIN, true>), grid, dim3(256), 0, st, a);
+      else hipLaunchKernelGGL((gemm_nt_kernel<WM, WN, TM, TN, MX_PLAIN>), grid, dim3(256), 0, st, a);
+      break;
     case MX_BNACT: hipLaunchKernelGGL((gemm_nt_kernel<WM, WN, TM, TN, MX_BNACT>), grid, dim3(256), 0, st, a); break;
     case MX_BNBWD: hipLaunchKernelGGL((gemm_nt_kernel<WM, WN, TM, TN, MX_BNBWD>), grid, dim3(256), 0, st, a); break;
     default: hipLaunchKernelGGL((gemm_nt_kernel<WM, WN, TM, TN, MX_AFFINE>), grid, dim3(256), 0, st, a); break;
@@ -1172,6 +1297,32 @@
   }
 }
 
+struct Pool5Req { const float* x; const float* a; const float* b; float* part; int rps; long bytes; };
+static thread_local Pool5Req t_pool5{};
+static Pool5Req take_pool5() {
+  const Pool5Req r = t_pool5;
+  t_pool5 = Pool5Req{};
+  return r;
+}
+static long pool5_bytes(int M, int N, int rps) { return ((long)cdiv(M, 128) + M / rps) * 5 * N * (long)sizeof(float); }
+static bool pool5_shape_ok(int M, int N, int rps) {
+  return M > 0 && N > 0 && rps >= 128 && M % rps == 0 && N % 4 == 0 && (long)M + rps < 0x7fffffffL;
+}
+static int apply_pool5(GemmArgs& g, const Pool5Req& r, int batch) {
+  MX_CHECK_ARG(batch == 1 && g.a.mode == MX_PLAIN && !g.bias && !g.residual && !g.relu && !g.stats,
+               "gemm: the pool5 epilogue takes a plain, unbatched launch without bias / residual / relu / statistics");
+  MX_CHECK_ARG(g.ldc == g.N, "gemm: the pool5 epilogue needs a contiguous output (ldc=%d, N=%d)", g.ldc, g.N);
+  MX_CHECK_ARG(pool5_shape_ok(g.M, g.N, r.rps),
+               "gemm: the pool5 epilogue cannot take M=%d N=%d rows_per_sample=%d (whole samples of >= 128 rows, N a multiple of 4)", g.M, g.N, r.rps);
+  MX_CHECK_ARG(r.bytes >= pool5_bytes(g.M, g.N, r.rps), "gemm: pool5 partial buffer of %ld bytes required (mx_pw_pool5_bytes)", pool5_bytes(g.M, g.N, r.rps));
+  g.pool_x = r.x; g.pool_a = r.a; g.pool_b = r.b; g.pool_part = r.part; g.pool_rps = r.rps;
+  return MX_OK;
+}
+#define MX_NO_POOL5(name)                                                                                      \
+  do {                                                                                                         \
+    if (take_pool5().x) MX_CHECK_ARG(false, name ": a pool5 epilogue request is pending and this launch cannot honour it"); \
+  } while (0)
+
 static int check_operand(const MxOperand& o, const char* nm) {
   MX_CHECK_ARG(o.p != nullptr, "gemm: operand %s is null", nm);
   MX_CHECK_ARG(((uintptr_t)o.p & 15) == 0, "gemm: operand %s not 16-byte aligned", nm);
@@ -1197,6 +1348,7 @@
 }
 
 static int gemm_common(int layout, GemmArgs& g, int batch, hipStream_t st) {
+  const Pool5Req pool = layout == L_NT ? take_pool5() : Pool5Req{};
   if (int e = check_operand(g.a, "A")) return e;
   if (int e = check_operand(g.b, "B")) return e;
   MX_CHECK_ARG(g.c != nullptr, "gemm: C is null");
@@ -1206,6 +1358,11 @@
   g.stamps = mx_gemm_stamps;
   if (layout == L_NT) {
     MX_CHECK_ARG(g.K % 4 == 0, "gemm NT: K=%d must be a multiple of 4", g.K);
+    if (pool.x) {
+      MX_CHECK_ARG(g.b.mode == MX_PLAIN && !(g.a.mode != MX_BNBWD && nt_uses_split(g.N, g.K)),
+                   "gemm NT: the first-generation split kernel has no pool5 epilogue (N=%d K=%d)", g.N, g.K);
+      if (int e = apply_pool5(g, pool, batch)) return e;
+    }
     if (g.b.mode == MX_PLAIN) dispatch_nt(g, batch, st);
     else dispatch<L_NT>(g, batch, st);
   } else if (layout == L_NN) {
@@ -1318,6 +1475,7 @@
 
 int mx_pw_fwd_planes(const float* A, const void* Wplanes, float* C, int M, int K, int N, int lda, int ldc,
                      const float* bias, const float* residual, int relu, float* stats, void* stream) {
+  const Pool5Req pool = take_pool5();
   MX_CHECK_ARG(A && Wplanes && C, "pw_fwd_planes: null pointer");
   MX_CHECK_ARG(M > 0 && N > 0 && K > 0 && K % 16 == 0, "pw_fwd_planes: bad extents M=%d N=%d K=%d (K must be a multiple of 16)", M, N, K);
   MX_CHECK_ARG(lda % 4 == 0 && lda >= K && ldc >= N, "pw_fwd_planes: bad leading dimensions lda=%d ldc=%d", lda, ldc);
@@ -1328,6 +1486,9 @@
   g.c = C; g.M = M; g.N = N; g.K = K; g.lda = lda; g.ldb = (N + 127) & ~127; g.ldc = ldc;
   g.bias = bias; g.residual = residual; g.relu = relu; g.stats = stats;
   g.stamps = mx_gemm_stamps;
+  if (pool.x) {
+    if (int e = apply_pool5(g, pool, 1)) return e;
+  }
   launch_nt_split3(g, 1, (hipStream_t)stream);
   MX_LAUNCH_CHECK();
   return MX_OK;
@@ -1339,6 +1500,7 @@
 
 int mx_pw_fwd_planes_act(const float* A, const float* scale, const float* shift, const float* gate, int rows_per_sample,
                          const void* Wplanes, float* C, int M, int K, int N, int lda, int ldc, float* stats, void* stream) {
+  MX_NO_POOL5("pw_fwd_planes_act");
   MX_CHECK_ARG(A && scale && shift && gate && Wplanes && C, "pw_fwd_planes_act: null pointer");
   MX_CHECK_ARG(M > 0 && N > 0 && K > 0 && K % 32 == 0 && rows_per_sample > 0, "pw_fwd_planes_act: bad extents M=%d N=%d K=%d rows_per_sample=%d", M, N, K, rows_per_sample);
   MX_CHECK_ARG(lda % 4 == 0 && lda >= K && ldc >= N, "pw_fwd_planes_act: bad leading dimensions lda=%d ldc=%d", lda, ldc);
@@ -1356,6 +1518,7 @@
 
 int mx_pw_dgrad_bnbwd_planes(const float* G, const float* X, const float* coef, const void* WtPlanes, float* dX, int M, int K, int N,
                              int ldg, int ldx, const float* residual, void* stream) {
+  MX_NO_POOL5("pw_dgrad_bnbwd_planes");
   MX_CHECK_ARG(G && X && coef && WtPlanes && dX, "pw_dgrad_bnbwd_planes: null pointer");
   MX_CHECK_ARG(M > 0 && N > 0 && K > 0 && K % 32 == 0, "pw_dgrad_bnbwd_planes: bad extents M=%d N=%d K=%d (K must be a multiple of 32)", M, N, K);
   MX_CHECK_ARG(ldg % 4 == 0 && ldg >= K && ldx >= N, "pw_dgrad_bnbwd_planes: bad leading dimensions");
@@ -1370,6 +1533,22 @@
   return MX_OK;
 }
 
+long mx_pw_pool5_bytes(int planes, int M, int K, int N, int rows_per_sample) {
+  if (M <= 0 || K <= 0 || N <= 0 || rows_per_sample <= 0) return MX_EARG;
+  if (planes ? K % 16 != 0 : (K % 4 != 0 || nt_uses_split(N, K))) return 0;
+  return pool5_shape_ok(M, N, rows_per_sample) ? pool5_bytes(M, N, rows_per_sample) : 0;
+}
+
+int mx_pw_epilogue_pool5(const float* X, const float* scale, const float* shift, int rows_per_sample, float* part5, long bytes) {
+  t_pool5 = Pool5Req{};
+  if (!X && !scale && !shift && !part5) return MX_OK;
+  MX_CHECK_ARG(X && scale && shift && part5 && rows_per_sample >= 128 && bytes > 0,
+               "pw_epilogue_pool5: bad arguments (rows_per_sample=%d must be >= 128)", rows_per_sample);
+  MX_CHECK_ARG((((uintptr_t)X | (uintptr_t)scale | (uintptr_t)shift | (uintptr_t)part5) & 15) == 0, "pw_epilogue_pool5: pointers must be 16-byte aligned");
+  t_pool5 = Pool5Req{X, scale, shift, part5, rows_per_sample, bytes};
+  return MX_OK;
+}
+
 int mx_set_gemm_mode(int mode) {
   MX_CHECK_ARG(mode >= 0 && mode <= 2, "set_gemm_mode: mode %d (0 fp32 MFMA, 1 split for MFMA-bound shapes, 2 split everywhere)", mode);
   g_gemm_mode = mode;
@@ -1414,6 +1593,7 @@
 
 int mx_pw_dgrad_bnbwd(const float* G, const float* X, const float* coef, const float* Wt, float* dX, float* dZ, int M, int K, int N,
                       int ldg, int ldx, const float* residual, void* stream) {
+  MX_NO_POOL5("pw_dgrad_bnbwd");
   MX_CHECK_ARG(G && X && coef && Wt && dX && dZ, "pw_dgrad_bnbwd: null pointer");
   MX_CHECK_ARG(dZ != G && dZ != X, "pw_dgrad_bnbwd: dZ must not alias G or X (other N tiles still read them)");
   MX_CHECK_ARG((((uintptr_t)X | (uintptr_t)dZ | (uintptr_t)coef) & 15) == 0 && K % 4 == 0, "pw_dgrad_bnbwd: alignment");
diff --git a/muscle_amd/engine.py b/muscle_amd/engine.py
--- a/muscle_amd/engine.py
+++ b/muscle_amd/engine.py
@@ -309,6 +309,9 @@
 
 FOLD_BN0_EARLY = os.environ.get("MUSCLE_FOLD_BN0_EARLY", "1") == "1"
 DW_S2_FUSED = os.environ.get("MUSCLE_DW_S2_FUSED", "1") == "1"
+SE_POOL_FUSED = os.environ.get("MUSCLE_SE_POOL_FUSED", "1") == "1"
+SE_POOL_FUSED_MIN_ROWS = 4096
+SE_POOL_FUSED_MAX_CEXP = int(os.environ.get("MUSCLE_SE_POOL_FUSED_MAX_CEXP", "288"))
 WGRAD_SIDE_STREAM = os.environ.get("MUSCLE_WGRAD_STREAM", "1") == "1"
 _side_streams: Dict[int, "torch.cuda.Stream"] = {}
 
@@ -365,6 +368,11 @@
 
 def _dw_input(t: BlockTape):
     return (t.e_raw, t.bn0) if t.cfg.expand else (t.x, t.x_st)
+
+
+def _se_pool_fused(Mo, cout, cexp, hw, planes) -> bool:
+    return (SE_POOL_FUSED and Mo >= SE_POOL_FUSED_MIN_ROWS and cexp <= SE_POOL_FUSED_MAX_CEXP
+            and ops.pw_pool5_takes(Mo, cout, cexp, hw, planes is not None))
 
 
 def _project_backward(lane, tape: Tape, t: BlockTape, m, g_out, sink: GradSink):
@@ -378,16 +386,20 @@
     else:
         lane.wgrad(dp, t.d_raw.view(Mo, b.cexp), sink.of(m._project_conv.weight).view(b.cout, b.cexp), x_mode=ops.BNACT,
                    x_scale=t.bn1.scale, x_shift=t.bn1.shift, x_gate=t.gate, rows_per_sample=hw)
+    planes = tape.wtp.get(id(m._project_conv.weight))
+    pool5 = (t.d_raw.view(Mo, b.cexp), t.bn1, hw) if _se_pool_fused(Mo, b.cout, b.cexp, hw, planes) else None
+    kw = {} if pool5 is None else {"pool5": pool5}
     ga = ops.pw_dgrad(dp, m._project_conv.weight.view(b.cout, b.cexp), b.cexp, wt=tape.wt.get(id(m._project_conv.weight)),
-                      planes=tape.wtp.get(id(m._project_conv.weight)))
+                      planes=planes, **kw)
     lane.flush()
-    return ga
-
-
-def _se_bn1_coeffs(tape: Tape, t: BlockTape, m, ga, sink: GradSink):
+    return ga if pool5 is not None else (ga, None)
+
+
+def _se_bn1_coeffs(tape: Tape, t: BlockTape, m, ga, sink: GradSink, pooled5=None):
     b, hw = t.cfg, t.Ho * t.Wo
     Mo = tape.N * hw
-    pooled5 = ops.se_bn1_pool(ga, t.d_raw.view(Mo, b.cexp), t.bn1, hw)
+    if pooled5 is None:
+        pooled5 = ops.se_bn1_pool(ga, t.d_raw.view(Mo, b.cexp), t.bn1, hw)
     gh = ops.se_bwd(pooled5[0], t.gate, t.s, t.h, m._se_expand.weight.view(b.cexp, b.se),
                     sink.of(m._se_reduce.weight).view(b.se, b.cexp), sink.of(m._se_reduce.bias),
                     sink.of(m._se_expand.weight).view(b.cexp, b.se), sink.of(m._se_expand.bias))
@@ -456,8 +468,9 @@
             g_out = tg if g_out is None else g_out + tg
         if g_out is None:
             continue
-        ga = _project_backward(lane, tape, t, m, g_out, sink)
-        c1, add = _se_bn1_coeffs(tape, t, m, ga, sink)
+        ga, pooled5 = _project_backward(lane, tape, t, m, g_out, sink)
+        c1, add = _se_bn1_coeffs(tape, t, m, ga, sink, pooled5)
+        del pooled5
         skip_res = g_out if t.cfg.skip else None
         gx, part0 = _depthwise_backward(lane, tape, t, m, ga, c1, add, skip_res, sink)
         del ga
diff --git a/muscle_amd/ops.py b/muscle_amd/ops.py
--- a/muscle_amd/ops.py
+++ b/muscle_amd/ops.py
@@ -206,19 +206,47 @@
     return out
 
 
-def pw_dgrad(G, W, N_in, *, residual=None, out=None, wt=None, planes=None):
+def pw_pool5_takes(M, K, N_in, rows_per_sample, planes=True):
+    if K % 4:
+        return False
+    use_planes = bool(planes) and _planes_take(M, K, N_in)
+    return lib().mx_pw_pool5_bytes(int(use_planes), M, K, N_in, rows_per_sample) > 0
+
+
+def pw_dgrad(G, W, N_in, *, residual=None, out=None, wt=None, planes=None, pool5=None):
     M, K = G.shape
     if out is None:
         out = _f32(M, N_in, device=G.device)
     if K % 4 == 0:
-        if planes is not None and _planes_take(M, K, N_in):
-            call("mx_pw_fwd_planes", ptr(G), planes, ptr(out), M, K, N_in, G.stride(0), N_in, None, ptr(residual), 0, None, stream())
+        use_planes = planes is not None and _planes_take(M, K, N_in)
+        part = None
+        if pool5 is not None:
+            X2d, st, rps = pool5
+            nb = lib().mx_pw_pool5_bytes(int(use_planes), M, K, N_in, rps)
+            if nb <= 0 or residual is not None or tuple(X2d.shape) != (M, N_in) or not X2d.is_contiguous():
+                raise ValueError(f"pw_dgrad: no pool5 epilogue for M={M} K={K} N={N_in} rows_per_sample={rps}")
+            part = torch.empty(nb // 4, dtype=torch.float32, device=G.device)
+            call("mx_pw_epilogue_pool5", ptr(X2d), ptr(st.scale), ptr(st.shift), rps, ptr(part), nb)
+        try:
+            if use_planes:
+                call("mx_pw_fwd_planes", ptr(G), planes, ptr(out), M, K, N_in, G.stride(0), N_in, None, ptr(residual), 0, None, stream())
+            else:
+                wt_ = wt if wt is not None else transpose(W)
+                call("mx_pw_fwd", ptr(G), PLAIN, None, None, None, 1, ptr(wt_), ptr(out), M, K, N_in, G.stride(0), N_in,
+                     None, ptr(residual), 0, None, stream())
+        except Exception:
+            if part is not None:
+                call("mx_pw_epilogue_pool5", None, None, None, 0, None, 0)
+            raise
+        if pool5 is None:
             return out
-        call("mx_pw_fwd", ptr(G), PLAIN, None, None, None, 1, ptr(wt if wt is not None else transpose(W)), ptr(out), M, K, N_in, G.stride(0), N_in,
-             None, ptr(residual), 0, None, stream())
+        out5 = _f32(5, M // rps, N_in, device=G.device)
+        call("mx_se_pool5_join", ptr(part), M, N_in, rps, ptr(out5), stream())
+        return out, out5
+    call("mx_pw_dgrad", ptr(G), ptr(W), ptr(out), M, K, N_in, G.stride(0), N_in, ptr(residual), stream())
+    if pool5 is None:
         return out
-    call("mx_pw_dgrad", ptr(G), ptr(W), ptr(out), M, K, N_in, G.stride(0), N_in, ptr(residual), stream())
-    return out
+    return out, se_bn1_pool(out, *pool5)
 
 
 def pw_dgrad_bnbwd(G, X, coef, W, N_in, *, residual=None, wt=None):
```

After: 339.3 images/sec. No clear change (-0.0%).
